# facebookresearch/KeypointNeRF

Measured on AMD Instinct MI355X. Metric: rendered rays/sec (64 coarse + 64 fine samples/ray), higher is better.
Workload: dtype f32 (dominant kernel: every fp32 operand as two fp16 pieces (22 bits, the residual formed exactly), three fp16-MFMA products per term set (hh hl lh: all terms above 2^-24 relative), fp32 accumulation; everything else fp32)

## Files before the change

### include/kpnerf.h

```cpp
#ifndef KPNERF_H
#define KPNERF_H

#include <stddef.h>
#include <stdint.h>

#ifdef __cplusplus
extern "C" {
#endif

#define KPN_ABI_VERSION 10
#define KPN_N_KPT 24
#define KPN_MAX_VIEWS 16

enum { KPN_OK = 0, KPN_EINVAL = -1, KPN_ELAUNCH = -2, KPN_EWORKSPACE = -3 };

int kpn_abi_version(void);
const char* kpn_last_error(void);
int kpn_is_device_build(void);

size_t kpn_plain_weight_floats(void);
size_t kpn_packed_weight_floats(void);
int kpn_pack_weights(const float* plain_host, float* packed_host);
int kpn_pack_weights_device(const float* plain_dev, float* packed_dev, void* stream);

// ... 31 lines not shown

int kpn_importance_sample(const float* contrib, const float* z, const float* u, int64_t n_rays, int32_t d_minus_2,
                          int32_t n_samples, float* samples_out, void* stream);

int kpn_rgba2out(const float* rgba, const float* z, int64_t n_rays, int32_t n_samples, float* color, float* depth,
                 float* alpha, float* contrib, float* sdf, void* stream);

int kpn_rgba2out_backward(const float* rgba, const float* z, int64_t n_rays, int32_t n_samples, const float* d_color,
                          const float* d_depth, const float* d_alpha, const float* d_sdf, float* d_rgba, void* stream);

size_t kpn_geo_rows_backward_workspace_bytes(int64_t n_points, int32_t n_views);
int kpn_geo_rows_backward(const kpn_scene_desc* desc, const void* scene_ws, const float* packed_weights, int64_t n_points,
                          const float* pts, uint32_t keep_mask, const float* d_x, float* d_plain, float* d_geo0,
                          float* d_geo1, void* workspace, size_t workspace_bytes, void* stream);

size_t kpn_query_backward_geometry_workspace_bytes(int64_t n_points, int32_t n_views);
int kpn_query_backward_geometry(const kpn_scene_desc* desc, const void* scene_ws, const float* packed_weights,
                                int64_t n_points, const float* pts, int32_t mode, uint32_t keep_mask, const float* noise,
                                float noise_std, const float* d_out, float* d_plain, float* d_geo0, float* d_geo1,
                                void* workspace, size_t workspace_bytes, void* stream);

size_t kpn_query_backward_workspace_bytes(int64_t n_points, int32_t n_views);
int kpn_query_backward(const kpn_scene_desc* desc, const void* scene_ws, const float* packed_weights, int64_t n_points,
                       const float* pts, const float* view, int32_t mode, uint32_t keep_mask, const float* noise,
                       float noise_std, const float* d_out, float* d_plain, float* d_geo0, float* d_geo1, float* d_tex,
                       void* workspace, size_t workspace_bytes, void* stream);

size_t kpn_geo_rows_backward_workspace_bytes_kpt(int64_t n_points, int32_t n_views);
int kpn_geo_rows_backward_kpt(const kpn_scene_desc* desc, const void* scene_ws, const float* packed_weights, int64_t n_points,
                              const float* pts, uint32_t keep_mask, const float* d_x, float* d_plain, float* d_geo0,
                              float* d_geo1, float* d_kpt3d, int32_t n_kpt, void* workspace, size_t workspace_bytes, void* stream);
size_t kpn_query_backward_workspace_bytes_kpt(int64_t n_points, int32_t n_views);
int kpn_query_backward_kpt(const kpn_scene_desc* desc, const void* scene_ws, const float* packed_weights, int64_t n_points,
                           const float* pts, const float* view, int32_t mode, uint32_t keep_mask, const float* noise,
                           float noise_std, const float* d_out, float* d_plain, float* d_geo0, float* d_geo1, float* d_tex,
                           float* d_kpt3d, int32_t n_kpt, void* workspace, size_t workspace_bytes, void* stream);

int kpn_set_geo_rows_mode(int32_t mode);
int kpn_get_geo_rows_mode(void);
int kpn_set_fuse_mode(int32_t mode);
int kpn_get_fuse_mode(void);
int kpn_set_density_first(int32_t mode);
int kpn_get_density_first(void);
int kpn_density_first_passes(int64_t* density_first, int64_t* fused, int32_t reset);
int kpn_density_stats(void* stream, int64_t* listed, int64_t* live, int32_t reset);
int kpn_packed_f16_range_check(const float* packed_weights_dev, void* stream, int32_t* beyond);
int kpn_set_range_guard(int32_t on);
int kpn_get_range_guard(void);
int kpn_range_guard_count(void* stream, int64_t* batches_host);

size_t kpn_query_workspace_bytes(int64_t n_points, int32_t n_views);
int kpn_query(const kpn_scene_desc* desc, const void* scene_ws, const float* packed_weights, int64_t n_points,
              const float* pts, const float* view, int32_t mode, float* out, uint8_t* valid, void* workspace,
              size_t workspace_bytes, void* stream);

typedef struct kpn_render_stages {
    float* z_coarse;
    float* rgba_coarse;
    float* z_fine;
    float* rgba_fine;
    float* dirs;
    float* cam_pos;
} kpn_render_stages;
typedef struct kpn_render_args {
    const float* K;
    const float* RT;
    const float* bounds;
    float znear, zfar;
    int32_t x0, y0, step, nx, ny;
    int32_t n_coarse, n_fine;
    int32_t fine;
    int32_t chunk_rays;
    float* tex_fg; float* depth; float* alpha;
    float* tex_fg_fine; float* depth_fine; float* alpha_fine; float* sdf;
    int32_t step_y;
    int32_t rows_kernel;
    int32_t fuse_kernel;
    const kpn_render_stages* stages;
} kpn_render_args;
enum { KPN_ROWS_DEFAULT = 0, KPN_ROWS_F32 = 1, KPN_ROWS_BF16X3 = 2, KPN_ROWS_F16X2 = 3 };
enum { KPN_FUSE_DEFAULT = 0, KPN_FUSE_F32 = 1, KPN_FUSE_F16X2 = 2 };

size_t kpn_render_workspace_bytes(const kpn_scene_desc* desc, const kpn_render_args* args);
int kpn_render_rays(const kpn_scene_desc* desc, const void* scene_ws, const float* packed_weights,
                    const kpn_render_args* args, void* workspace, size_t workspace_bytes, void* stream);

int kpn_pix_l1_loss(const float* src, const float* tar, int64_t n, float lambda, float* loss, float* d_src, void* scratch,
                    void* stream);
typedef struct kpn_train_loss_args {
    const float* tex;
    const float* tex_fine;
    const float* tar;
    const float* alpha;
    const float* alpha_fine;
    const float* tar_alpha;
    int64_t n;
    float l1_c, l1, l2, lp, mloss;
    int32_t reset_ticket;
    float* terms;
    float* d_tex;
    float* d_tex_fine;
    float* d_alpha;
    float* d_alpha_fine;
} kpn_train_loss_args;
size_t kpn_train_loss_workspace_bytes(int64_t n);
int kpn_train_loss(const kpn_train_loss_args* args, void* workspace, void* stream);
int kpn_frame_to_rgb8(const float* chw, int32_t height, int32_t width, int32_t bgr, uint8_t* hwc_out, void* stream);
int kpn_mse_psnr(const float* pred, const float* gt, int64_t n, double* out2, void* scratch, void* stream);
size_t kpn_ssim_scratch_bytes(int32_t crop_w, int32_t crop_h);
int kpn_ssim(const float* pred_chw, const float* gt_chw, int32_t height, int32_t width, int32_t x0, int32_t y0, int32_t crop_w,
             int32_t crop_h, double* out, void* scratch, void* stream);

int kpn_profile_enable(int32_t on);
int kpn_profile_collect(double* geo_rows_ms_host, int64_t* launches_host, int64_t* rows_host);
int kpn_profile_collect2(double* geo_rows_ms_host, int64_t* launches_host, int64_t* rows_host, int64_t* surplus_launches_host);
int kpn_profile_collect3(double* geo_rows_ms_host, int64_t* launches_host, int64_t* rows_host, int64_t* surplus_launches_host,
                         double* clock_ghz_host);
int kpn_bwd_profile_enable(int32_t on);
int kpn_bwd_profile_collect(double* ms5, int64_t* launches5, int64_t* rows, int64_t* kept_rows, int64_t* points);
size_t kpn_row_scratch_cap_bytes(void);
int kpn_set_row_scratch_cap_bytes(size_t bytes);

typedef struct kpn_train_args {
    const int32_t* pix;
    const float* u_coarse;
    const float* noise_coarse;
    const float* noise_fine;
    const float* u_fine;
    uint32_t keep_coarse;
    uint32_t keep_fine;
    float rand_noise_std;
} kpn_train_args;
int kpn_render_rays_train(const kpn_scene_desc* desc, const void* scene_ws, const float* packed_weights,
                          const kpn_render_args* args, const kpn_train_args* train, void* workspace,
                          size_t workspace_bytes, void* stream);

typedef struct kpn_render_grads {
    const float* d_tex_fg; const float* d_depth; const float* d_alpha;
    const float* d_tex_fg_fine; const float* d_depth_fine; const float* d_alpha_fine; const float* d_sdf;
} kpn_render_grads;
size_t kpn_render_rays_train_backward_workspace_bytes(const kpn_scene_desc* desc, const kpn_render_args* args);
int kpn_render_rays_train_backward(const kpn_scene_desc* desc, const void* scene_ws, const float* packed_weights,
                                   const kpn_render_args* args, const kpn_train_args* train, const kpn_render_grads* grads,
                                   float* d_plain, float* d_geo0, float* d_geo1, float* d_tex, void* workspace,
                                   size_t workspace_bytes, void* stream);

size_t kpn_render_rays_train_state_bytes(const kpn_scene_desc* desc, const kpn_render_args* args);
int kpn_render_rays_train_keep(const kpn_scene_desc* desc, const void* scene_ws, const float* packed_weights,
                               const kpn_render_args* args, const kpn_train_args* train, void* state, size_t state_bytes,
                               void* stream);
int kpn_render_rays_train_backward_kept(const kpn_scene_desc* desc, const void* scene_ws, const float* packed_weights,
                                        const kpn_render_args* args, const kpn_train_args* train, const kpn_render_grads* grads,
                                        float* d_plain, float* d_geo0, float* d_geo1, float* d_tex, void* state,
                                        size_t state_bytes, void* workspace, size_t workspace_bytes, void* stream);

size_t kpn_render_rays_train_backward_workspace_bytes_kpt(const kpn_scene_desc* desc, const kpn_render_args* args);
int kpn_render_rays_train_backward_kpt(const kpn_scene_desc* desc, const void* scene_ws, const float* packed_weights,
                                       const kpn_render_args* args, const kpn_train_args* train, const kpn_render_grads* grads,
                                       float* d_plain, float* d_geo0, float* d_geo1, float* d_tex, float* d_kpt3d, int32_t n_kpt,
                                       void* workspace, size_t workspace_bytes, void* stream);
int kpn_render_rays_train_backward_kept_kpt(const kpn_scene_desc* desc, const void* scene_ws, const float* packed_weights,
                                            const kpn_render_args* args, const kpn_train_args* train, const kpn_render_grads* grads,
                                            float* d_plain, float* d_geo0, float* d_geo1, float* d_tex, float* d_kpt3d,
                                            int32_t n_kpt, void* state, size_t state_bytes, void* workspace,
                                            size_t workspace_bytes, void* stream);

// ... 216 lines not shown
```

### keypointnerf_amd/csrc/api_backward.hip

```cpp
namespace {
const int64_t kBwdChunk = 262144;
static_assert(kBwdChunk <= 262144, "kUncappedPoints (query_layout) must cover a backward pass");
#ifndef KPN_GRAD_WORKERS
#define KPN_GRAD_WORKERS 512
#endif
const int kGradWorkers = kEmu ? 3 : KPN_GRAD_WORKERS;
const int kPartialUnits = 72;
struct BwdBufs { kpn_bwd_bufs B; kpn_fuse_bwd_bufs F; kpn_color_bufs C; };
enum { PART_GEO = 0, PART_FUSE, PART_DXROWS, PART_COLOR, PART_CMP };
const int kPartFull[5] = {0, 1, 1, 2, 2};
enum { U_X0 = 0, U_X1, U_X2, U_X3, U_D0, U_D1, U_D2, U_D3, U_XP, U_XH0, U_XH1, U_D20, U_D21, U_D22, U_DXROWS,
       U_XRD, U_XE1, U_XDIR, U_XBL, U_XB1, U_XA, U_XV10, U_XV11, U_XT33, U_XV20, U_XV21, U_XO0, U_XO1, U_XO2,
       U_DO2, U_DO1, U_DO0, U_DV21, U_DV20, U_DV11, U_DV10, U_DBL1, U_DBL0, U_DRE1, U_DRE0, U_DCMP, U_COUNT };
struct Dump { int id; size_t member; int ld; int part; };
#define D(id, member, ld, part) {U_##id, offsetof(BwdBufs, member), ld, PART_##part}
constexpr Dump kDumps[U_COUNT] = {
    D(X0, B.X0, KPN_LDX0, GEO), D(X1, B.X1, 128, GEO), D(X2, B.X2, KPN_LDX2, GEO), D(X3, B.X3, 128, GEO),
    D(D0, B.D0, 128, GEO), D(D1, B.D1, 128, GEO), D(D2, B.D2, 128, GEO), D(D3, B.D3, 64, GEO),
    D(XP, F.Xp, 128, FUSE), D(XH0, F.Xh0, 64, FUSE), D(XH1, F.Xh1, 64, FUSE), D(D20, F.D20, 64, FUSE), D(D21, F.D21, 64, FUSE), D(D22, F.D22, 2, FUSE),
    D(DXROWS, F.dxrows, 64, DXROWS),
    D(XRD, C.Xrd, 4, COLOR), D(XE1, C.Xe1, 16, COLOR), D(XDIR, C.Xdir, KPN_LD_XDIR, COLOR), D(XBL, C.Xbl, KPN_LD_XBL, COLOR), D(XB1, C.Xb1, 64, COLOR),
    D(XA, C.Xa, 32, COLOR), D(XV10, C.Xv10, 32, COLOR), D(XV11, C.Xv11, 32, COLOR), D(XT33, C.Xt33, 2, COLOR), D(XV20, C.Xv20, 32, COLOR),
    D(XV21, C.Xv21, 32, COLOR), D(XO0, C.Xo0, KPN_LD_XO0, COLOR), D(XO1, C.Xo1, 16, COLOR), D(XO2, C.Xo2, 8, COLOR),
    D(DO2, C.Do2, 2, COLOR), D(DO1, C.Do1, 8, COLOR), D(DO0, C.Do0, 16, COLOR), D(DV21, C.Dv21, 2, COLOR), D(DV20, C.Dv20, 32, COLOR),
// ... 97 lines not shown
    if (p.ws_bytes < L.total) return fail(KPN_EWORKSPACE, "backward workspace too small");
    const KptLayout K = kpt_layout(L.total, V);
    if (p.d_kpt) {
        KPN_REQUIRE(p.n_kpt >= 1 && p.n_kpt <= KPN_NKPT, "n_kpt in 1..24");
        if (p.ws_bytes < K.total) return fail(KPN_EWORKSPACE, "backward workspace too small for the keypoint gradient");
    }
    if (p.marched && p.N > L.chunk) return fail(KPN_EINVAL, "ray-marched backward pass too large");
    kpn_scene_dev sc = scene_dev(d, scene_ws);
    sc.keep = p.keep_mask;
    char* base = static_cast<char*>(p.ws);
    auto fp = [&](size_t off) { return reinterpret_cast<float*>(base + off); };
    int* count = reinterpret_cast<int*>(base + L.count);
    int64_t* rows_dev = reinterpret_cast<int64_t*>(base + L.count + 64);
    int* list = reinterpret_cast<int*>(base + L.list);
    BwdBufs u{};
    for (const Dump& m : kDumps) if (full >= kPartFull[m.part]) dump_slot(u, m) = fp(L.dump[m.id]);
    u.B.dgeo0 = p.d_geo0; u.B.dgeo1 = p.d_geo1;
    if (full == 2) {
        u.C.dtex = p.d_tex;
        u.C.dani = p.d_plain + kpn_plain_weight_floats() - 1;
        u.F.Dcmp = u.C.Dcmp;
    }
    const int blocks = field_grid_blocks();
    const uint32_t wgrad_keep = p.keep_mask | ~((V >= 32) ? 0xFFFFFFFFu : ((1u << V) - 1u));
    kpn_wgrad_jobs jobs[3], all;
    int gzmax[3];
    size_t partial_used = 0;
    bool overflow = false;
    auto queue_jobs = [&](int stage) {
        for (const WgradRow& r : kWgrad) {
            if (r.stage != stage) continue;
            const Dump &dy = kDumps[r.dY], &x = kDumps[r.X];
            const int cls = r.mv == 1 ? 0 : (r.mv == 2 ? 1 : 2);
            const int gz = (r.Kc + 63) / 64;
            kpn_wgrad_job j;
            j.dY = dump_slot(u, dy); j.X = dump_slot(u, x); j.ldy = dy.ld; j.M = r.M; j.ldx = x.ld; j.Kc = r.Kc; j.Kt = r.Kt;
            j.cmap = r.cmap; j.omap = r.omap; j.mv = r.mv;
            j.which = per_point(x) ? 1 : 0;
            j.V = per_point(x) ? 1 : V; j.keep = per_point(x) ? 0xFFFFFFFFu : wgrad_keep;
            j.partial = fp(L.partial) + partial_used;
            partial_used += (size_t)gz * kGradWorkers * r.mv * 2048;
            if (partial_used > (size_t)kPartialUnits * kGradWorkers * 2048 || all.n >= KPN_WGRAD_MAX_JOBS) { overflow = true; continue; }
            j.dbp = fp(L.dbp) + (size_t)all.n * kGradWorkers * 4 * 64;
            j.dW = p.d_plain + plain_w_off(r.layer);
            j.dB = p.d_plain + plain_b_off(r.layer);
            j.in_dim = plain_dims[r.layer][1];
            jobs[cls].j[jobs[cls].n++] = j;
            all.j[all.n++] = j;
            if (gz > gzmax[cls]) gzmax[cls] = gz;
        }
    };
    auto run_jobs = [&]() {
        if (jobs[0].n) KPN_LAUNCH(k_weight_grad<1>, dim3(kGradWorkers, jobs[0].n), dim3(64 * gzmax[0]), stream, jobs[0], (const int64_t*)rows_dev);
        if (jobs[1].n) KPN_LAUNCH(k_weight_grad<2>, dim3(kGradWorkers, jobs[1].n), dim3(64 * gzmax[1]), stream, jobs[1], (const int64_t*)rows_dev);
        if (jobs[2].n) KPN_LAUNCH(k_weight_grad<4>, dim3(kGradWorkers, jobs[2].n), dim3(64 * gzmax[2]), stream, jobs[2], (const int64_t*)rows_dev);
        int gz_all = gzmax[0] > gzmax[1] ? gzmax[0] : gzmax[1];
        if (gzmax[2] > gz_all) gz_all = gzmax[2];
        const int mv_all = jobs[2].n ? 4 : (jobs[1].n ? 2 : 1);
        if (all.n) KPN_LAUNCH(k_weight_grad_reduce, dim3((mv_all * 2048 + mv_all * 32 + 31) / 32, gz_all, all.n), dim3(256), stream, all,
                              (int)kGradWorkers);
    };
    if (p.d_kpt) {
        hipMemsetAsync(base + K.partial, 0, K.partial_bytes, (hipStream_t)stream);
        KPN_LAUNCH(k_kpt_grad_pack, grid1d(KPN_KG_WT_FLOATS, 256), dim3(256), stream, wp, fp(K.wt));
    }
    for (int64_t c0 = 0; c0 < p.N; c0 += L.chunk) {
        const int64_t n = (p.N - c0 < L.chunk) ? (p.N - c0) : L.chunk;
        const kpn_points ps = p.marched ? *p.marched
                                        : kpn_points{p.pts + c0 * 3, (p.view ? p.view : p.pts) + c0 * 3, nullptr, nullptr, nullptr, 1,
                                                     p.noise ? p.noise + c0 : nullptr, p.noise_std};
        jobs[0].n = jobs[1].n = jobs[2].n = all.n = 0; gzmax[0] = gzmax[1] = gzmax[2] = 0; partial_used = 0;
        hipMemsetAsync(count, 0, 8 * sizeof(int), (hipStream_t)stream);
        const int* vcount = count;
        float* xscr = full ? fp(L.xscr) : nullptr;
        if (p.fwd_query_ws && full) {
            const QueryLayout Q = query_layout(n, V);
            char* qb = static_cast<char*>(p.fwd_query_ws);
            vcount = reinterpret_cast<const int*>(qb + Q.count);
            list = reinterpret_cast<int*>(qb + Q.list);
            xscr = reinterpret_cast<float*>(qb + Q.xscr);
        } else {
            const int ppt = mask_points_per_thread(n);
            KPN_LAUNCH(k_mask_compact, grid1d(n, 256 * ppt), dim3(256), stream, sc, ps, n, 0, 1, ppt, wp + kpn_scalar_off(), (float*)nullptr,
                       (uint8_t*)nullptr, list, count);
        }
        KPN_LAUNCH(k_bwd_rows, dim3(1), dim3(1), stream, vcount, V, rows_dev);
        bwd_prof_pass(vcount, V, p.keep_mask, stream);
        if (full) {
            if (!p.fwd_query_ws) {
                KPN_BPROF(BP_ROWS_FWD);
                KPN_LAUNCH(k_geo_rows, dim3(blocks), dim3(256), stream, sc, ps, wp, (const int*)list, vcount, count + 1, xscr,
                           kpn_batch{0, 1 << 30});
            }
            if (full == 2) {
                KPN_BPROF(BP_COLOR_BWD);
                if (V <= 3)
                    KPN_LAUNCH(k_color_bwd<3>, dim3(blocks), dim3(256), stream, sc, ps, wp, (const int*)list, vcount, count + 4,
                               (const float*)xscr, p.d_out + c0 * 5, u.C);
                else
                    KPN_LAUNCH(k_color_bwd<KPN_MAXV>, dim3(blocks), dim3(256), stream, sc, ps, wp, (const int*)list, vcount, count + 4,
                               (const float*)xscr, p.d_out + c0 * 5, u.C);
            }
            if (full == 2) queue_jobs(ST_COLOR);
            {
                KPN_BPROF(BP_FUSE_BWD);
                KPN_LAUNCH(k_fuse_bwd, dim3(blocks), dim3(256), stream, sc, ps, wp, (const int*)list, vcount, count + 2,
                           (const float*)xscr, p.mode, p.d_out + c0 * 5, u.F);
            }
            queue_jobs(ST_LAYERS2);
            if (full == 2) queue_jobs(ST_COMPRESS);
        }
        {
            KPN_BPROF(BP_ROWS_BWD);
            KPN_LAUNCH(k_geo_rows_bwd, dim3(blocks), dim3(256), stream, sc, ps, wp, (const int*)list, vcount, count + 3,
                       full ? (const float*)u.F.dxrows : p.d_x + c0 * V * 64, full ? 1 : 0, u.B);
        }
        if (p.d_kpt) {
            const kpn_kpt_grad_args ka{u.B.D0, u.B.X0, fp(K.wt), reinterpret_cast<double*>(base + K.partial), p.n_kpt, wgrad_keep};
            KPN_LAUNCH(k_kpt_grad, dim3(kKptWorkers, V), dim3(256), stream, sc, ps, (const int*)list, vcount, ka);
        }
        queue_jobs(ST_LAYERS1);
        if (overflow) return fail(KPN_EWORKSPACE, "weight-gradient scratch too small (internal)");
        {
            KPN_BPROF(BP_WGRAD);
            run_jobs();
        }
    }
    if (p.d_kpt)
        KPN_LAUNCH(k_kpt_grad_finish, dim3(p.n_kpt), dim3(256), stream, sc, (const double*)reinterpret_cast<double*>(base + K.partial),
                   (int)kKptWorkers, p.d_kpt);
    return check_launch("field backward");
}
}

extern "C" size_t kpn_geo_rows_backward_workspace_bytes(int64_t N, int32_t V) { return bwd_workspace_bytes(N, V, 0); }

extern "C" int kpn_geo_rows_backward(const kpn_scene_desc* d, const void* scene_ws, const float* wp, int64_t N,
                                     const float* pts, uint32_t keep_mask, const float* d_x, float* d_plain, float* d_geo0,
                                     float* d_geo1, void* ws, size_t ws_bytes, void* stream) {
    if (int e = check_desc(d)) return e;
    KPN_REQUIRE(N >= 0 && N < (1ll << 31), "point count out of range");
    if (N == 0) return KPN_OK;
    KPN_REQUIRE(scene_ws && wp && pts && d_x && d_plain && d_geo0 && d_geo1 && ws, "null pointer");
    BackwardPass p;
    p.N = N; p.pts = pts; p.keep_mask = keep_mask; p.d_x = d_x;
    p.d_plain = d_plain; p.d_geo0 = d_geo0; p.d_geo1 = d_geo1; p.ws = ws; p.ws_bytes = ws_bytes;
    return run_backward(d, scene_ws, wp, p, stream);
}

extern "C" size_t kpn_geo_rows_backward_workspace_bytes_kpt(int64_t N, int32_t V) { return bwd_workspace_bytes_kpt(N, V, 0); }

extern "C" int kpn_geo_rows_backward_kpt(const kpn_scene_desc* d, const void* scene_ws, const float* wp, int64_t N,
                                         const float* pts, uint32_t keep_mask, const float* d_x, float* d_plain, float* d_geo0,
                                         float* d_geo1, float* d_kpt3d, int32_t n_kpt, void* ws, size_t ws_bytes, void* stream) {
    if (int e = check_desc(d)) return e;
    KPN_REQUIRE(N >= 0 && N < (1ll << 31), "point count out of range");
    KPN_REQUIRE(n_kpt >= 1 && n_kpt <= KPN_NKPT, "n_kpt in 1..24");
    if (N == 0) return KPN_OK;
    KPN_REQUIRE(scene_ws && wp && pts && d_x && d_plain && d_geo0 && d_geo1 && d_kpt3d && ws, "null pointer");
    BackwardPass p;
    p.N = N; p.pts = pts; p.keep_mask = keep_mask; p.d_x = d_x;
    p.d_plain = d_plain; p.d_geo0 = d_geo0; p.d_geo1 = d_geo1; p.ws = ws; p.ws_bytes = ws_bytes;
    p.d_kpt = d_kpt3d; p.n_kpt = n_kpt;
    return run_backward(d, scene_ws, wp, p, stream);
}

extern "C" size_t kpn_query_backward_geometry_workspace_bytes(int64_t N, int32_t V) { return bwd_workspace_bytes(N, V, 1); }
// ... 52 lines not shown
```

### keypointnerf_amd/csrc/api_field.hip

```cpp
namespace {
struct Setting { long long value = -1; template <class Init> long long get(Init init) { if (value < 0) value = init(); return value; } };
bool env_flag(const char* name) { const char* e = getenv(name); return e && atoi(e) != 0; }
#ifdef KPN_SIMT_EMU
const bool kEmu = true;
#else
const bool kEmu = false;
#endif
Setting g_row_scratch_cap, g_geo_rows_mode, g_fuse_mode, g_density_first, g_range_guard, g_no_pool;

size_t row_scratch_cap_bytes() {
    return (size_t)g_row_scratch_cap.get([] {
        const char* e = getenv("KPN_ROW_SCRATCH_MIB");
        return (long long)((e ? (size_t)atoll(e) : (size_t)(kEmu ? 1 : 3072)) << 20);
    });
}
const int kMaxBatches = 60;
const size_t kCounterBytes = 2048;
static_assert((8 + 8 * kMaxBatches) * sizeof(int) <= kCounterBytes && kCounterBytes % 256 == 0, "counter block");
const int64_t kUncappedPoints = kEmu ? 2048 : 262144;
struct QueryLayout { size_t count, list, live, xscr, total; int tiles_cap, nbatch; };
#ifndef KPN_DEFAULT_GEO_ROWS_MODE
#define KPN_DEFAULT_GEO_ROWS_MODE 3
#endif
int geo_rows_mode() { return (int)g_geo_rows_mode.get([] { return (long long)KPN_DEFAULT_GEO_ROWS_MODE; }); }
// ... 43 lines not shown
    return &g_density_hint[0];
#endif
}
long long g_density_first_passes[2] = {0, 0};
bool density_first_now() {
    const int m = density_first();
    if (m != 2) return m == 1;
    DensityHint* hnt = density_hint();
    if (!hnt) return false;
#ifndef KPN_SIMT_EMU
    if (!hnt->pinned) return hnt->split;
    const unsigned long long now[2] = {hnt->pinned[0], hnt->pinned[1]};
#else
    const unsigned long long now[2] = {kpn_density_counts[0], kpn_density_counts[1]};
#endif
    const bool was_reset = now[0] < hnt->seen[0];
    const unsigned long long d0 = was_reset ? now[0] : now[0] - hnt->seen[0], d1 = was_reset ? now[1] : now[1] - hnt->seen[1];
    if (d0 > 0 && d1 <= d0) {
        hnt->avg[0] = 0.5 * hnt->avg[0] + (double)d0;
        hnt->avg[1] = 0.5 * hnt->avg[1] + (double)d1;
        hnt->split = (hnt->avg[0] - hnt->avg[1]) >= (double)kDensityFirstDeadFraction * hnt->avg[0];
        hnt->seen[0] = now[0]; hnt->seen[1] = now[1];
    }
    return hnt->split;
}
void density_hint_refresh(void* stream) {
#ifndef KPN_SIMT_EMU
    if (density_first() != 2 || stream_is_capturing(stream)) return;
    DensityHint* hnt = density_hint();
    if (!hnt) return;
    if (!hnt->pinned) {
        void* hp = nullptr;
        if (hipHostMalloc(&hp, 2 * sizeof(unsigned long long), hipHostMallocDefault) != hipSuccess) { (void)hipGetLastError(); return; }
        hnt->pinned = static_cast<unsigned long long*>(hp);
        hnt->pinned[0] = hnt->pinned[1] = 0;
    }
    void* dp = nullptr;
    if (hipGetSymbolAddress(&dp, HIP_SYMBOL(kpn_density_counts)) != hipSuccess) { (void)hipGetLastError(); return; }
    (void)hipMemcpyAsync(hnt->pinned, dp, 2 * sizeof(unsigned long long), hipMemcpyDeviceToHost, (hipStream_t)stream);
#else
    (void)stream;
#endif
}
int pair_grid_blocks() {
#ifdef KPN_SIMT_EMU
    return 8;
#else
    static int blocks = [] {
        int dev = 0, cus = 0;
        if (hipGetDevice(&dev) != hipSuccess || hipDeviceGetAttribute(&cus, hipDeviceAttributeMultiprocessorCount, dev) != hipSuccess || cus <= 0) cus = 256;
        return cus;
    }();
    return blocks;
#endif
}
int fuse_grid_blocks() { return kEmu ? 4 : 256; }
int records_grid_blocks() { return kEmu ? 8 : 2048; }
static inline int mask_points_per_thread(int64_t N) {
    const int64_t min_groups = kEmu ? 2 : 2048;
    int ppt = KPN_MASK_PPT;
    while (ppt > 1 && N / (256 * (int64_t)ppt) < min_groups) ppt >>= 1;
    return ppt;
}
int range_guard() { return (int)g_range_guard.get([] { return (long long)!env_flag("KPN_NO_RANGE_GUARD"); }); }
#ifndef KPN_SIMT_EMU
__device__ int kpn_redone_batches;
#else
static int kpn_redone_batches;
#endif
int* redone_counter() {
#ifndef KPN_SIMT_EMU
    void* p = nullptr;
    if (hipGetSymbolAddress(&p, HIP_SYMBOL(kpn_redone_batches)) != hipSuccess) return nullptr;
    return static_cast<int*>(p);
#else
    return &kpn_redone_batches;
#endif
}

struct FieldPass {
    kpn_points points; int64_t N = 0; int mode = 0;
    float* out = nullptr; uint8_t* valid = nullptr; void* ws = nullptr;
    bool lean = false, keep_rows = false, allow_pool = false; int rows_sel = 0, fuse_sel = 0;
};
struct FieldLaunch { const kpn_scene_dev& sc; const kpn_points& ps; const float* wp; int *list, *count, *live; float* xscr; void* stream; };
kpn_batch make_batch(int index, int tiles_cap, bool pool, int cond = KPN_RUN_ALWAYS, int* bad = nullptr, int* redone = nullptr) {
    return kpn_batch{index, tiles_cap, cond, bad, redone, pool ? 1 : 0, nullptr};
}

void launch_rows(const FieldLaunch& f, int rows_mode, int* tickets, const kpn_batch& batch) {
    if (rows_mode >= 2)
        kpn_internal_launch_geo_rows_pair(rows_mode, pair_grid_blocks(), f.stream, &f.sc, &f.ps, f.wp, f.list, f.count, tickets, f.xscr, &batch);
    else
        KPN_LAUNCH(k_geo_rows, dim3(field_grid_blocks()), dim3(256), f.stream, f.sc, f.ps, f.wp, (const int*)f.list, (const int*)f.count, tickets, f.xscr, batch);
}
void launch_records(const FieldLaunch& f, const kpn_batch& batch) {
    kpn_internal_launch_row_records(records_grid_blocks(), f.stream, &f.sc, &f.ps, f.wp, f.list, f.count, f.xscr, &batch);
}
bool use_h3(const kpn_scene_dev& sc) { return sc.V == 3 && (sc.keep & 7u) == 7u && !env_flag("KPN_NO_FUSE_H3"); }
void launch_fuse(const FieldLaunch& f, int fmode, int* tickets, int mode, float* out, const kpn_batch& batch, int zero_skip) {
    auto* kernel = fmode != 1 ? k_fuse_color : (use_h3(f.sc) ? k_fuse_color_h3 : k_fuse_color_h);
    KPN_LAUNCH(kernel, dim3(fuse_grid_blocks()), dim3(512), f.stream, f.sc, f.ps, f.wp, (const int*)f.list, (const int*)f.count, tickets, (const float*)f.xscr, mode, 0, out, batch, zero_skip);
}
void launch_density_first(const FieldLaunch& f, int* tickets, float* out, const kpn_batch& batch) {
    const int fblocks = fuse_grid_blocks();
    KPN_LAUNCH(k_density_h, dim3(fblocks), dim3(512), f.stream, f.sc, f.ps, f.wp, (const int*)f.list, (const int*)f.count, tickets, f.xscr, f.live, out, batch);
    kpn_internal_launch_row_records_live(records_grid_blocks(), f.stream, &f.sc, &f.ps, f.wp, f.list, f.count, tickets, f.live, f.xscr, &batch);
    auto* colour = use_h3(f.sc) ? k_colour_h3 : k_colour_h;
    KPN_LAUNCH(colour, dim3(fblocks), dim3(512), f.stream, f.sc, f.ps, f.wp, (const int*)f.list, (const int*)f.count, tickets, (const float*)f.xscr, f.live, out, batch);
}

int selected_rows_mode(int sel) { return sel == KPN_ROWS_F32 ? 0 : (sel == KPN_ROWS_BF16X3 ? 2 : (sel == KPN_ROWS_F16X2 ? 3 : geo_rows_mode())); }
int selected_fuse_mode(int sel) { return sel == KPN_FUSE_F32 ? 0 : (sel == KPN_FUSE_F16X2 ? 1 : fuse_mode()); }

int run_field(const kpn_scene_dev& sc, const float* wp, const FieldPass& p, void* stream) {
    const kpn_points& ps = p.points;
    const int rmode = selected_rows_mode(p.rows_sel);
    const int fmode = !p.out ? 0 : selected_fuse_mode(p.fuse_sel);
    const bool pool = p.allow_pool && !p.keep_rows && p.out && pool_layout_selected() && rmode >= 2;
    const QueryLayout L = query_layout(p.N, sc.V, pool);
    char* base = static_cast<char*>(p.ws);
    int* count = reinterpret_cast<int*>(base + L.count);
    const FieldLaunch f{sc, ps, wp, reinterpret_cast<int*>(base + L.list), count, reinterpret_cast<int*>(base + L.live),
                        reinterpret_cast<float*>(base + L.xscr), stream};
    hipMemsetAsync(count, 0, kCounterBytes, (hipStream_t)stream);
    const int ppt = mask_points_per_thread(p.N);
    KPN_LAUNCH(k_mask_compact, grid1d(p.N, 256 * ppt), dim3(256), stream, sc, ps, p.N, p.mode, (int)p.lean, ppt, wp + kpn_scalar_off(), p.out, p.valid, f.list, count);
    if (p.keep_rows && L.nbatch > 1) return fail(KPN_EWORKSPACE, "a pass whose rows a backward call reads again must fit the row scratch");
    const bool guard = range_guard() && p.out && (rmode == 3 || fmode == 1);
    int* redone = guard ? redone_counter() : nullptr;
    const int safe_rmode = rmode == 3 ? 2 : rmode;
    auto guarded = [&](bool f16) { return guard && f16 ? KPN_RUN_IF_SAFE : KPN_RUN_ALWAYS; };
    const int zero_skip = (p.lean && !p.keep_rows && !env_flag("KPN_NO_ZERO_SKIP")) ? 1 : 0;
    const bool eligible = zero_skip && p.mode == 1 && ps.noise == nullptr && pool && fmode == 1;
    const bool split = eligible && density_first_now();
    if (eligible) ++g_density_first_passes[split ? 0 : 1];
    for (int b = 0; b < L.nbatch; ++b) {
        int* slots = count + 8 + 8 * b;
        int* bad = guard ? slots + 6 : nullptr;
        kpn_batch b_rows = make_batch(b, L.tiles_cap, pool, guarded(rmode == 3), bad);
        {
            KPN_FPROF(b_rows, rmode >= 2, count, sc.V);
            launch_rows(f, rmode, slots + 0, b_rows);
        }
        if (rmode >= 2 && !split) launch_records(f, make_batch(b, L.tiles_cap, pool));
        if (!p.out) continue;
        const kpn_batch b_fuse = make_batch(b, L.tiles_cap, pool, guarded(fmode == 1), bad);
        if (split) launch_density_first(f, slots, p.out, b_fuse);
        else launch_fuse(f, fmode, slots, p.mode, p.out, b_fuse, zero_skip);
        if (guard) {
            const kpn_batch r_rows = make_batch(b, L.tiles_cap, pool, KPN_RUN_IF_UNSAFE, bad);
            launch_rows(f, safe_rmode, slots + 4, r_rows);
            if (split) launch_records(f, r_rows);
            launch_fuse(f, 0, slots + 4, p.mode, p.out, make_batch(b, L.tiles_cap, pool, KPN_RUN_IF_UNSAFE, bad, redone), zero_skip);
        }
    }
    if (eligible) density_hint_refresh(stream);
    return check_launch("field query");
}
}

extern "C" int kpn_set_geo_rows_mode(int32_t mode) {
    KPN_REQUIRE(mode == 0 || mode == 2 || mode == 3, "mode must be 0 (fp32 MFMA), 2 (three bf16 pieces) or 3 (two fp16 pieces); mode 1 is not part of the library");
    g_geo_rows_mode.value = mode;
    return KPN_OK;
}
extern "C" int kpn_get_geo_rows_mode(void) { return geo_rows_mode(); }
extern "C" int kpn_set_fuse_mode(int32_t mode) {
    KPN_REQUIRE(mode == 0 || mode == 1, "mode must be 0 (fp32 MFMA) or 1 (two fp16 pieces per operand)");
    g_fuse_mode.value = mode;
    return KPN_OK;
}
extern "C" int kpn_get_fuse_mode(void) { return fuse_mode(); }
extern "C" int kpn_density_stats(void* stream, int64_t* listed_host, int64_t* live_host, int32_t reset) {
    KPN_REQUIRE(listed_host && live_host, "null pointer");
    unsigned long long v[2] = {0, 0};
#ifndef KPN_SIMT_EMU
    void* p = nullptr;
    if (hipGetSymbolAddress(&p, HIP_SYMBOL(kpn_density_counts)) != hipSuccess) return fail(KPN_ELAUNCH, "no density counters in this module");
    if (hipMemcpyAsync(v, p, sizeof(v), hipMemcpyDeviceToHost, (hipStream_t)stream) != hipSuccess ||
        (reset && hipMemsetAsync(p, 0, sizeof(v), (hipStream_t)stream) != hipSuccess) ||
        hipStreamSynchronize((hipStream_t)stream) != hipSuccess) return fail(KPN_ELAUNCH, "could not read the density counters");
#else
    (void)stream;
    v[0] = kpn_density_counts[0]; v[1] = kpn_density_counts[1];
    if (reset) kpn_density_counts[0] = kpn_density_counts[1] = 0;
#endif
    *listed_host = (int64_t)v[0];
    *live_host = (int64_t)v[1];
    return KPN_OK;
}
#if defined(KPN_PRECISION_PROBE) && !defined(KPN_SIMT_EMU)
extern "C" int kpn_internal_probe_set_mask_pair(unsigned long long m);
extern "C" int kpn_probe_set_mask(unsigned long long m) {
    if (hipMemcpyToSymbol(HIP_SYMBOL(kpn_probe_mask_dev), &m, sizeof(m)) != hipSuccess) return fail(KPN_ELAUNCH, "probe mask");
    if (kpn_internal_probe_set_mask_pair(m)) return fail(KPN_ELAUNCH, "probe mask (pair unit)");
    return hipDeviceSynchronize() == hipSuccess ? KPN_OK : KPN_ELAUNCH;
}
#endif
extern "C" int kpn_density_first_passes(int64_t* density_first_host, int64_t* fused_host, int32_t reset) {
    KPN_REQUIRE(density_first_host && fused_host, "null pointer");
    *density_first_host = g_density_first_passes[0];
    *fused_host = g_density_first_passes[1];
    if (reset) g_density_first_passes[0] = g_density_first_passes[1] = 0;
    return KPN_OK;
}
extern "C" int kpn_set_density_first(int32_t mode) {
    KPN_REQUIRE(mode >= 0 && mode <= 2, "mode must be 0 (fused per-point kernel), 1 (density first) or 2 (auto)");
    g_density_first.value = mode;
    return KPN_OK;
// ... 47 lines not shown
```

### keypointnerf_amd/csrc/api_render.hip

```cpp
namespace {
struct RayBlock { size_t cam_pos, dirs, nearv, farv; };
struct RayView { float *cam_pos, *dirs, *nearv, *farv; };
RayBlock carve_rays(Carver& c, int64_t R) { return {c.take(64), c.take((size_t)R * 3 * 4), c.take((size_t)R * 4), c.take((size_t)R * 4)}; }
struct ChunkBlock { size_t zc, zf, rgba_c, rgba_f, contrib, query_c, query_f; };
struct ChunkView { float *zc, *zf, *rgba_c, *rgba_f, *contrib; char *query_c, *query_f; };
ChunkBlock carve_chunk(Carver& c, int64_t C, int64_t Sc, int64_t Sfull, bool train) {
    ChunkBlock k{};
    k.zc = c.take((size_t)C * Sc * 4); k.zf = c.take((size_t)C * Sfull * 4);
    if (train) {
        k.rgba_c = c.take((size_t)C * Sc * 5 * 4); k.rgba_f = c.take((size_t)C * Sfull * 5 * 4);
        k.contrib = c.take((size_t)C * (Sfull > 8 ? Sfull : 8) * 4);
    } else {
        k.rgba_c = k.rgba_f = c.take((size_t)C * Sfull * 5 * 4);
        c.o += 256;
    }
    return k;
}
template <class T = float> T* at(void* base, size_t off) { return reinterpret_cast<T*>(static_cast<char*>(base) + off); }
RayView ray_view(void* base, const RayBlock& r) { return {at(base, r.cam_pos), at(base, r.dirs), at(base, r.nearv), at(base, r.farv)}; }
ChunkView chunk_view(void* base, const ChunkBlock& k) {
    return {at(base, k.zc), at(base, k.zf), at(base, k.rgba_c), at(base, k.rgba_f), at(base, k.contrib), at<char>(base, k.query_c), at<char>(base, k.query_f)};
}

struct RenderLayout { RayBlock rays; ChunkBlock k; size_t rgba_n, zn, src, color, depth, alpha, sdf, total; int64_t chunk; };
int64_t pick_chunk(const kpn_scene_desc* d, const kpn_render_args* a) {
    const int64_t R = (int64_t)a->nx * a->ny;
    int64_t c = a->chunk_rays;
    if (c <= 0) {
        const int64_t cmax = 262144;
        const int64_t npass = (R + cmax - 1) / cmax;
        c = ((R + npass - 1) / npass + 63) / 64 * 64;
    }
    return c < R ? c : R;
}
RenderLayout render_layout(const kpn_scene_desc* d, const kpn_render_args* a) {
    RenderLayout L;
    const int64_t C = pick_chunk(d, a);
    const int64_t Sfull = a->n_coarse + (a->fine ? a->n_fine : 0);
    Carver c;
    L.chunk = C;
    L.rays = carve_rays(c, (int64_t)a->nx * a->ny);
    L.k = carve_chunk(c, C, a->n_coarse, Sfull, false);
    L.rgba_n = L.k.rgba_c + align_up((size_t)C * a->n_coarse * 5 * 4, 256);
    L.zn = c.take((size_t)C * (a->fine ? a->n_fine : 0) * 4);
    L.src = c.take((size_t)C * Sfull * sizeof(int16_t));
    L.k.contrib = c.take((size_t)C * a->n_coarse * 4);
    L.color = c.take((size_t)C * 3 * 4);
    L.depth = c.take((size_t)C * 4);
    L.alpha = c.take((size_t)C * 4);
    L.sdf = c.take((size_t)C * 4);
    {
        const size_t qa = query_layout(C * Sfull, d->n_views, false).total, qb = query_layout(C * Sfull, d->n_views, pool_layout_selected()).total;
        L.k.query_c = L.k.query_f = c.take(qa > qb ? qa : qb);
    }
    L.total = c.o;
    return L;
}
int check_render(const kpn_render_args* a) {
    KPN_REQUIRE(a != nullptr, "render args null");
    KPN_REQUIRE(a->K && a->RT && a->bounds, "null camera/bounds");
    KPN_REQUIRE(a->nx > 0 && a->ny > 0 && a->step > 0 && a->step_y >= 0, "bad pixel grid");
    KPN_REQUIRE(a->rows_kernel >= 0 && a->rows_kernel <= KPN_ROWS_F16X2 && a->fuse_kernel >= 0 && a->fuse_kernel <= KPN_FUSE_F16X2, "bad kernel selection");
    KPN_REQUIRE(a->n_coarse >= 3 && a->n_coarse <= 128, "sample_per_ray_c must be in [3,128]");
    KPN_REQUIRE(!a->fine || (a->n_fine >= 1 && a->n_fine <= 128), "sample_per_ray_f must be in [1,128]");
    KPN_REQUIRE((int64_t)a->nx * a->ny < (1ll << 31), "too many rays");
    return KPN_OK;
}
int check_train(const kpn_scene_desc* d, const kpn_render_args* a, const kpn_train_args* t, bool need_fine) {
    KPN_REQUIRE(t != nullptr, "train args null");
    KPN_REQUIRE(a->fine || !need_fine, "the train branch renders coarse + fine (dr_kwargs.fine)");
    KPN_REQUIRE(t->pix && t->u_coarse, "train args: pix and u_coarse are required");
    KPN_REQUIRE(!a->fine || t->u_fine, "train args: u_fine is required when fine");
    KPN_REQUIRE(t->rand_noise_std == 0.0f || (t->noise_coarse && (!a->fine || t->noise_fine)), "train args: noise tensors missing");
    KPN_REQUIRE((t->keep_coarse & ((1u << d->n_views) - 1u)) && (t->keep_fine & ((1u << d->n_views) - 1u)),
                "train args: view dropout must keep at least one view (reference src/model.py:744)");
    return KPN_OK;
}
}

__global__ void k_store_planar(int64_t r0, int64_t n, int64_t R, int C, const float* __restrict__ src, float* __restrict__ dst) {
    const int64_t i = (int64_t)blockIdx.x * blockDim.x + threadIdx.x;
    if (i >= n * C) return;
    const int64_t r = i / C;
    const int c = (int)(i - r * C);
    dst[(int64_t)c * R + r0 + r] = src[i];
}
__global__ void k_load_planar(int64_t r0, int64_t n, int64_t R, int C, const float* __restrict__ src, float* __restrict__ dst) {
    const int64_t i = (int64_t)blockIdx.x * blockDim.x + threadIdx.x;
    if (i >= n * C) return;
    const int64_t r = i / C;
    const int c = (int)(i - r * C);
    dst[i] = src ? src[(int64_t)c * R + r0 + r] : 0.0f;
}
struct PlanarChunk {
    void* stream; int64_t r0, n, R;
    void store(float* dst, const float* src, int C) const {
        if (dst) KPN_LAUNCH(k_store_planar, grid1d(n * C, 256), dim3(256), stream, r0, n, R, C, src, dst);
    }
    void load(float* dst, const float* src, int C) const {
        KPN_LAUNCH(k_load_planar, grid1d(n * C, 256), dim3(256), stream, r0, n, R, C, src, dst);
    }
};

extern "C" size_t kpn_render_workspace_bytes(const kpn_scene_desc* d, const kpn_render_args* a) {
    if (check_desc(d) != KPN_OK || check_render(a) != KPN_OK) return 0;
    return render_layout(d, a).total;
}

static void launch_fine_samples(void* stream, int64_t n, int Sc, int Sf, const float* zc, const float* contrib,
                                const float* u, float* zf, float* znew, int16_t* src) {
    const bool small = Sc <= 64 && Sf <= 64;
    const int64_t per = 4 * KPN_FINE_GROUP(small);
    const dim3 grid((unsigned)((n + per - 1) / per < 8192 ? (n + per - 1) / per : 8192));
    if (small)
        KPN_LAUNCH(k_fine_samples_w<true>, grid, dim3(256), stream, n, Sc, Sf, zc, contrib, u, zf, znew, src);
    else
        KPN_LAUNCH(k_fine_samples_w<false>, grid, dim3(256), stream, n, Sc, Sf, zc, contrib, u, zf, znew, src);
}

static void launch_make_rays(void* stream, const kpn_render_args* a, const int* pix, int step_y, const RayView& rays) {
    KPN_LAUNCH(k_make_rays, grid1d((int64_t)a->nx * a->ny, 256), dim3(256), stream, a->K, a->RT, a->znear, a->zfar, a->bounds, (int)a->x0, (int)a->y0,
               (int)a->step, step_y, (int)a->nx, (int)a->ny, pix, rays.dirs, rays.cam_pos, rays.nearv, rays.farv);
}

static int render_impl(const kpn_scene_desc* d, const void* scene_ws, const float* wp, const kpn_render_args* a,
                       const kpn_train_args* t, void* ws, size_t ws_bytes, void* stream) {
    if (int e = check_desc(d)) return e;
    if (int e = check_render(a)) return e;
    KPN_REQUIRE(scene_ws && wp && ws, "null pointer");
    if (t) if (int e = check_train(d, a, t, false)) return e;
    const RenderLayout L = render_layout(d, a);
    if (ws_bytes < L.total) return fail(KPN_EWORKSPACE, "render workspace too small");
    const RayView rays = ray_view(ws, L.rays);
    const ChunkView k = chunk_view(ws, L.k);
    float *rgba_n = at(ws, L.rgba_n), *zn = at(ws, L.zn), *color = at(ws, L.color), *depth = at(ws, L.depth), *alpha = at(ws, L.alpha), *sdf = at(ws, L.sdf);
    int16_t* src = at<int16_t>(ws, L.src);
    kpn_scene_dev sc = scene_dev(d, scene_ws);
    const int64_t R = (int64_t)a->nx * a->ny;
    const int Sc = a->n_coarse, Sf = a->fine ? a->n_fine : 0, Sfull = Sc + Sf;
    const float std_ = t ? t->rand_noise_std : 0.0f;
    launch_make_rays(stream, a, t ? (const int*)t->pix : (const int*)nullptr, (int)(a->step_y > 0 ? a->step_y : a->step), rays);
    for (int64_t r0 = 0; r0 < R; r0 += L.chunk) {
        const int64_t n = (R - r0) < L.chunk ? (R - r0) : L.chunk;
        const float* dirs = rays.dirs + r0 * 3;
        const PlanarChunk pl{stream, r0, n, R};
        KPN_LAUNCH(k_coarse_z, grid1d(n * Sc, 256), dim3(256), stream, n, Sc, (const float*)(rays.nearv + r0),
                   (const float*)(rays.farv + r0), t ? t->u_coarse + r0 * Sc : (const float*)nullptr, k.zc);
        const bool reuse = (t == nullptr) && a->fine && !env_flag("KPN_NO_COARSE_REUSE");
        auto field = [&](const float* z, int S, const float* noise, float* out) {
            FieldPass p;
            p.points = kpn_points{nullptr, nullptr, rays.cam_pos, dirs, z, S, noise, std_};
            p.N = n * S; p.mode = 1; p.out = out; p.ws = k.query_c; p.lean = true; p.allow_pool = t == nullptr;
            p.rows_sel = a->rows_kernel; p.fuse_sel = a->fuse_kernel;
            return run_field(sc, wp, p, stream);
        };
        sc.keep = t ? t->keep_coarse : 0xFFFFFFFFu;
        if (int e = field(k.zc, Sc, std_ != 0.0f ? t->noise_coarse + r0 * Sc : nullptr, k.rgba_c)) return e;
        if (int e = kpn_rgba2out(k.rgba_c, k.zc, n, Sc, color, depth, alpha, k.contrib, sdf, stream)) return e;
        const kpn_render_stages* st = a->stages;
        auto copy_out = [&](float* dst, const float* src_, size_t floats) {
            (void)hipMemcpyAsync(dst, src_, floats * sizeof(float), hipMemcpyDeviceToDevice, (hipStream_t)stream);
        };
        if (st && st->dirs) copy_out(st->dirs + r0 * 3, dirs, (size_t)n * 3);
        if (st && st->cam_pos && r0 == 0) copy_out(st->cam_pos, rays.cam_pos, 3);
        if (st && st->z_coarse) copy_out(st->z_coarse + r0 * Sc, k.zc, (size_t)n * Sc);
        if (st && st->rgba_coarse) copy_out(st->rgba_coarse + r0 * Sc * 5, k.rgba_c, (size_t)n * Sc * 5);
        pl.store(a->tex_fg, color, 3);
        pl.store(a->depth, depth, 1);
        pl.store(a->alpha, alpha, 1);
        if (!a->fine) continue;
        launch_fine_samples(stream, n, Sc, Sf, k.zc, k.contrib, t ? t->u_fine + r0 * Sf : (const float*)nullptr, k.zf, reuse ? zn : nullptr,
                            reuse ? src : nullptr);
        sc.keep = t ? t->keep_fine : 0xFFFFFFFFu;
        if (reuse) {
            if (int e = field(zn, Sf, nullptr, rgba_n)) return e;
            if (int e = rgba2out_merged(k.rgba_c, rgba_n, src, k.zf, n, Sc, Sf, color, depth, alpha, sdf, stream)) return e;
        } else {
            if (int e = field(k.zf, Sfull, std_ != 0.0f ? t->noise_fine + r0 * Sfull : nullptr, k.rgba_f)) return e;
            if (int e = kpn_rgba2out(k.rgba_f, k.zf, n, Sfull, color, depth, alpha, nullptr, sdf, stream)) return e;
        }
        if (st && st->z_fine) copy_out(st->z_fine + r0 * Sfull, k.zf, (size_t)n * Sfull);
        if (st && st->rgba_fine) {
            if (reuse) KPN_LAUNCH(k_merge_rgba, grid1d(n * Sfull, 256), dim3(256), stream, n, Sfull, Sc, (const float*)k.rgba_c, (const float*)rgba_n,
                                  (const int16_t*)src, st->rgba_fine + r0 * Sfull * 5);
            else copy_out(st->rgba_fine + r0 * Sfull * 5, k.rgba_f, (size_t)n * Sfull * 5);
        }
        pl.store(a->tex_fg_fine, color, 3);
        pl.store(a->depth_fine, depth, 1);
        pl.store(a->alpha_fine, alpha, 1);
        pl.store(a->sdf, sdf, 1);
    }
    return check_launch("kpn_render_rays");
}

extern "C" int kpn_render_rays(const kpn_scene_desc* d, const void* scene_ws, const float* wp, const kpn_render_args* a,
                               void* ws, size_t ws_bytes, void* stream) {
    return render_impl(d, scene_ws, wp, a, nullptr, ws, ws_bytes, stream);
}
extern "C" int kpn_render_rays_train(const kpn_scene_desc* d, const void* scene_ws, const float* wp, const kpn_render_args* a,
                                     const kpn_train_args* t, void* ws, size_t ws_bytes, void* stream) {
    KPN_REQUIRE(t != nullptr, "train args null");
    return render_impl(d, scene_ws, wp, a, t, ws, ws_bytes, stream);
}

namespace {
struct TrainBwdLayout { RayBlock rays; ChunkBlock k; size_t scratch, g3, g1a, g1b, g1c, drgba_c, drgba_f, bwd, total; int64_t chunk; };
TrainBwdLayout train_bwd_layout(const kpn_scene_desc* d, const kpn_render_args* a) {
    TrainBwdLayout L;
    const int64_t R = (int64_t)a->nx * a->ny;
    const int64_t Sfull = a->n_coarse + a->n_fine;
    int64_t C = a->chunk_rays > 0 ? a->chunk_rays : kBwdChunk / Sfull;
    if (C * Sfull > kBwdChunk) C = kBwdChunk / Sfull;
    if (C > R) C = R;
    L.chunk = C;
    Carver c;
    L.rays = carve_rays(c, R);
    L.k = carve_chunk(c, C, a->n_coarse, Sfull, true);
    L.scratch = c.take((size_t)C * 8 * 4);
    L.g3 = c.take((size_t)C * 3 * 4); L.g1a = c.take((size_t)C * 4); L.g1b = c.take((size_t)C * 4); L.g1c = c.take((size_t)C * 4);
    L.drgba_c = c.take((size_t)C * a->n_coarse * 5 * 4); L.drgba_f = c.take((size_t)C * Sfull * 5 * 4);
    L.k.query_c = L.k.query_f = c.take(query_layout(C * Sfull, d->n_views).total);
    L.bwd = c.take(bwd_layout(C * Sfull, d->n_views, 2).total);
    L.total = c.o;
    return L;
}

struct TrainStateLayout { RayBlock rays; size_t chunk0; ChunkBlock k; size_t chunk_bytes, total; int64_t chunk, nchunks; };
TrainStateLayout train_state_layout(const kpn_scene_desc* d, const kpn_render_args* a) {
    TrainStateLayout S;
    const int64_t R = (int64_t)a->nx * a->ny, C = train_bwd_layout(d, a).chunk;
    const int64_t Sfull = a->n_coarse + a->n_fine;
    S.chunk = C; S.nchunks = (R + C - 1) / C;
    Carver c;
    S.rays = carve_rays(c, R);
    S.chunk0 = c.o;
    c = Carver();
    S.k = carve_chunk(c, C, a->n_coarse, Sfull, true);
    S.k.query_c = c.take(query_layout(C * a->n_coarse, d->n_views).total);
    S.k.query_f = c.take(query_layout(C * Sfull, d->n_views).total);
    S.chunk_bytes = c.o;
    S.total = S.chunk0 + S.chunk_bytes * (size_t)S.nchunks;
    return S;
}

struct TrainPass { bool fine; kpn_points ps; uint32_t keep; float *z, *rgba; char* query; };
struct TrainChunk { int64_t r0, n; ChunkView v; PlanarChunk pl; TrainPass coarse, fine; };
struct TrainCall {
    const kpn_scene_desc* d; const void* scene_ws; const float* wp; const kpn_render_args* a; const kpn_train_args* t;
    const kpn_render_grads* g; float *d_plain, *d_geo0, *d_geo1, *d_tex;
    void *state, *ws, *stream;
    TrainBwdLayout L; TrainStateLayout S;
    kpn_scene_dev sc; int64_t R; int Sc, Sf, Sfull; RayView rays;
    float* d_kpt = nullptr; int n_kpt = 0;
    size_t bwd_bytes() const { return d_kpt ? kpt_layout(L.total - L.bwd, d->n_views).total : L.total - L.bwd; }
    int begin(size_t state_bytes, size_t ws_bytes, bool forward_only) {
        if (int e = check_desc(d)) return e;
        if (int e = check_render(a)) return e;
        KPN_REQUIRE(a->rows_kernel == KPN_ROWS_DEFAULT && a->fuse_kernel == KPN_FUSE_DEFAULT,
                    "the train branch takes the process-wide kernel selection: rows_kernel / fuse_kernel must be 0");
        KPN_REQUIRE(scene_ws && wp, "null pointer");
        if (int e = check_train(d, a, t, true)) return e;
        if (!forward_only) KPN_REQUIRE(g && d_plain && d_geo0 && d_geo1 && d_tex && ws, "gradient pointers / workspace null");
        if (forward_only) KPN_REQUIRE(state != nullptr, "state null");
        L = train_bwd_layout(d, a);
        S = train_state_layout(d, a);
        if (d_kpt) KPN_REQUIRE(n_kpt >= 1 && n_kpt <= KPN_NKPT, "n_kpt in 1..24");
        if (!forward_only && ws_bytes < L.bwd + bwd_bytes()) return fail(KPN_EWORKSPACE, "train backward workspace too small");
        if (state && state_bytes < S.total) return fail(KPN_EWORKSPACE, "train state too small");
        sc = scene_dev(d, scene_ws);
// ... 138 lines not shown
```

### keypointnerf_amd/csrc/api_scene.hip

```cpp
namespace {
struct SceneLayout { size_t table, rgbm, geo0, geo1, tex, flags, total; };
SceneLayout scene_layout(const kpn_scene_desc* d) {
    SceneLayout L;
    Carver c;
    L.table = c.take((size_t)d->n_views * KPN_TBL_STRIDE, 64);
    L.rgbm = c.take((size_t)d->n_views * d->src_h * d->src_w * 4, 64);
    L.geo0 = c.take((size_t)d->n_views * d->geo0_h * d->geo0_w * 64, 64);
    L.geo1 = c.take((size_t)d->n_views * d->geo1_h * d->geo1_w * 8, 64);
    L.tex = c.take((size_t)d->n_views * d->tex_h * d->tex_w * 8, 64);
    L.flags = c.take((size_t)KPN_SCENE_FLAG_FLOATS, 64);
    L.total = c.o;
    return L;
}
int check_desc(const kpn_scene_desc* d) {
    KPN_REQUIRE(d != nullptr, "scene desc is null");
    KPN_REQUIRE(d->n_views >= 1 && d->n_views <= KPN_MAX_VIEWS, "n_views out of range");
    KPN_REQUIRE(d->src_h > 1 && d->src_w > 1 && d->geo0_h > 1 && d->geo0_w > 1 && d->geo1_h > 1 && d->geo1_w > 1 &&
                d->tex_h > 1 && d->tex_w > 1, "map sizes must be > 1");
    KPN_REQUIRE((int64_t)d->src_h * d->src_w <= INT32_MAX && (int64_t)d->geo0_h * d->geo0_w <= INT32_MAX &&
                (int64_t)d->geo1_h * d->geo1_w <= INT32_MAX && (int64_t)d->tex_h * d->tex_w <= INT32_MAX, "map too large");
    KPN_REQUIRE(d->zfar > d->znear && d->nml_scale > 0.0f && d->sigma > 0.0f, "bad scalar parameters");
    KPN_REQUIRE(d->KRT && d->extrin && d->kpt3d && d->img && d->geo0 && d->geo1 && d->tex, "null scene tensor");
    KPN_REQUIRE(d->disable_fg_mask || d->fg_mask, "fg_mask is null");
    return KPN_OK;
}
kpn_scene_dev scene_dev(const kpn_scene_desc* d, const void* ws) {
    const SceneLayout L = scene_layout(d);
    const float* base = static_cast<const float*>(ws);
    kpn_scene_dev s;
    s.V = d->n_views; s.H = d->src_h; s.W = d->src_w;
    s.g0h = d->geo0_h; s.g0w = d->geo0_w; s.g1h = d->geo1_h; s.g1w = d->geo1_w; s.th = d->tex_h; s.tw = d->tex_w;
    s.disable_fg_mask = d->disable_fg_mask;
    s.znear = d->znear; s.zfar = d->zfar; s.nml_scale = d->nml_scale;
    s.two_sigma2 = (float)(2.0 * ((double)d->sigma * (double)d->sigma));
    s.keep = 0xFFFFFFFFu;
    s.table = base + L.table; s.rgbm = base + L.rgbm; s.geo0 = base + L.geo0; s.geo1 = base + L.geo1; s.tex = base + L.tex;
    s.flags = base + L.flags;
    return s;
}
}

extern "C" size_t kpn_scene_workspace_bytes(const kpn_scene_desc* d) {
    if (check_desc(d) != KPN_OK) return 0;
    return scene_layout(d).total * sizeof(float);
}

extern "C" int kpn_scene_layout(const kpn_scene_desc* d, size_t offsets[6]) {
    if (int e = check_desc(d)) return e;
    KPN_REQUIRE(offsets != nullptr, "offsets is null");
    const SceneLayout L = scene_layout(d);
    offsets[0] = L.table; offsets[1] = L.rgbm; offsets[2] = L.geo0; offsets[3] = L.geo1; offsets[4] = L.tex; offsets[5] = L.flags;
    return KPN_OK;
}

extern "C" int kpn_scene_prepare(const kpn_scene_desc* d, void* scene_ws, void* stream) {
    return kpn_scene_prepare_kpt(d, KPN_NKPT, scene_ws, stream);
}

extern "C" int kpn_scene_prepare_kpt(const kpn_scene_desc* d, int32_t n_kpt, void* scene_ws, void* stream) {
    if (int e = check_desc(d)) return e;
    KPN_REQUIRE(n_kpt >= 1 && n_kpt <= KPN_NKPT, "n_kpt out of range: the field kernels hold 1..24 keypoints (KPN_N_KPT)");
    KPN_REQUIRE(scene_ws != nullptr, "scene workspace is null");
    const SceneLayout L = scene_layout(d);
    float* base = static_cast<float*>(scene_ws);
    const int V = d->n_views;
    float* flags = base + L.flags;
    KPN_LAUNCH(k_scene_table, dim3(V), dim3(128), stream, V, (int)n_kpt, d->KRT, d->extrin, d->kpt3d, base + L.table, flags);
    const int HW = d->src_h * d->src_w;
    const int ptiles = (HW + KPN_PACK_PIX - 1) / KPN_PACK_PIX;
    KPN_LAUNCH(k_pack_rgbm, dim3(V * ptiles), dim3(256), stream, HW, ptiles, d->img,
               d->disable_fg_mask ? (const uint8_t*)nullptr : d->fg_mask, base + L.rgbm, flags);
    auto vec = [](const float* p, int hw) { return (hw % 4 == 0 && reinterpret_cast<uintptr_t>(p) % 16 == 0) ? 1 : 0; };
    const int hw0 = d->geo0_h * d->geo0_w, hw1 = d->geo1_h * d->geo1_w, hwt = d->tex_h * d->tex_w;
    const int t0 = (hw0 + KPN_NHWC_TILE / 64 - 1) / (KPN_NHWC_TILE / 64), t1 = (hw1 + KPN_NHWC_TILE / 8 - 1) / (KPN_NHWC_TILE / 8),
              tt = (hwt + KPN_NHWC_TILE / 8 - 1) / (KPN_NHWC_TILE / 8);
    KPN_LAUNCH(k_nchw_to_nhwc<64>, dim3(V * t0), dim3(256), stream, hw0, t0, vec(d->geo0, hw0), d->geo0, base + L.geo0, flags);
    KPN_LAUNCH(k_nchw_to_nhwc<8>, dim3(V * t1), dim3(256), stream, hw1, t1, vec(d->geo1, hw1), d->geo1, base + L.geo1, flags);
    KPN_LAUNCH(k_nchw_to_nhwc<8>, dim3(V * tt), dim3(256), stream, hwt, tt, vec(d->tex, hwt), d->tex, base + L.tex, flags);
    return check_launch("kpn_scene_prepare");
}

extern "C" int kpn_ray_bbox_intersection(const float* bounds, const float* orig, const float* direct, int64_t R,
                                         float* near_o, float* far_o, uint8_t* hit_o, void* stream) {
    KPN_REQUIRE(bounds && orig && direct && near_o && far_o && hit_o, "null pointer");
    KPN_REQUIRE(R >= 0, "negative ray count");
    if (R == 0) return KPN_OK;
    KPN_LAUNCH(k_ray_bbox, grid1d(R, 256), dim3(256), stream, R, bounds, orig, direct, near_o, far_o, hit_o);
    return check_launch("kpn_ray_bbox_intersection");
}

extern "C" int kpn_make_rays(const float* K, const float* RT, float znear, float zfar, const float* bounds, int32_t x0,
                             int32_t y0, int32_t step, int32_t nx, int32_t ny, float* dirs, float* cam_pos,
                             float* near_o, float* far_o, void* stream) {
    KPN_REQUIRE(K && RT && bounds && dirs && cam_pos && near_o && far_o, "null pointer");
    KPN_REQUIRE(nx > 0 && ny > 0 && step > 0, "bad pixel grid");
    KPN_LAUNCH(k_make_rays, grid1d((int64_t)nx * ny, 256), dim3(256), stream, K, RT, znear, zfar, bounds, (int)x0, (int)y0,
               (int)step, (int)step, (int)nx, (int)ny, (const int*)nullptr, dirs, cam_pos, near_o, far_o);
    return check_launch("kpn_make_rays");
}

extern "C" int kpn_importance_sample(const float* contrib, const float* z, const float* u, int64_t R, int32_t Dm2,
                                     int32_t n, float* out, void* stream) {
    KPN_REQUIRE(contrib && z && out, "null pointer");
    KPN_REQUIRE(Dm2 >= 1 && Dm2 + 1 <= KPN_IS_MAXD, "bin count out of range (<= 128)");
    KPN_REQUIRE(n >= 1 && R >= 0, "bad sizes");
    if (R == 0) return KPN_OK;
    KPN_LAUNCH(k_importance, grid1d(R, 64), dim3(64), stream, R, (int)Dm2, (int)n, contrib, z, u, out);
    return check_launch("kpn_importance_sample");
}

static void launch_rgba2out(void* stream, int64_t R, int S, const float* rgba, const float* z, float* color, float* depth,
                            float* alpha, float* contrib, float* sdf, const int16_t* src, const float* rgba_new, int Sc) {
    const int64_t blocks = (R + 3) / 4;
    const dim3 grid((unsigned)(blocks < 8192 ? blocks : 8192));
    const int per = (S + 63) / 64;
    if (per <= 1) KPN_LAUNCH(k_rgba2out<1>, grid, dim3(256), stream, R, S, rgba, z, color, depth, alpha, contrib, sdf, src, rgba_new, Sc);
    else if (per <= 2) KPN_LAUNCH(k_rgba2out<2>, grid, dim3(256), stream, R, S, rgba, z, color, depth, alpha, contrib, sdf, src, rgba_new, Sc);
    else if (per <= 4) KPN_LAUNCH(k_rgba2out<4>, grid, dim3(256), stream, R, S, rgba, z, color, depth, alpha, contrib, sdf, src, rgba_new, Sc);
    else KPN_LAUNCH(k_rgba2out<KPN_MAX_PER_LANE>, grid, dim3(256), stream, R, S, rgba, z, color, depth, alpha, contrib, sdf, src, rgba_new, Sc);
}

extern "C" int kpn_rgba2out(const float* rgba, const float* z, int64_t R, int32_t S, float* color, float* depth,
                            float* alpha, float* contrib, float* sdf, void* stream) {
    KPN_REQUIRE(rgba && z && color && depth && alpha && sdf, "null pointer");
    KPN_REQUIRE(S >= 1 && S <= 64 * KPN_MAX_PER_LANE, "samples per ray out of range (<= 512)");
    if (R <= 0) return R == 0 ? KPN_OK : fail(KPN_EINVAL, "negative ray count");
    launch_rgba2out(stream, R, (int)S, rgba, z, color, depth, alpha, contrib, sdf, nullptr, nullptr, 0);
    return check_launch("kpn_rgba2out");
}
static int rgba2out_merged(const float* rgba_c, const float* rgba_n, const int16_t* src, const float* z, int64_t R, int Sc, int Sf,
                           float* color, float* depth, float* alpha, float* sdf, void* stream) {
    launch_rgba2out(stream, R, Sc + Sf, rgba_c, z, color, depth, alpha, nullptr, sdf, src, rgba_n, Sc);
    return check_launch("kpn_render_rays");
}

extern "C" int kpn_rgba2out_backward(const float* rgba, const float* z, int64_t R, int32_t S, const float* d_color,
                                     const float* d_depth, const float* d_alpha, const float* d_sdf, float* d_rgba, void* stream) {
    KPN_REQUIRE(rgba && z && d_rgba, "null pointer");
    KPN_REQUIRE(S >= 1, "bad sample count");
    if (R <= 0) return R == 0 ? KPN_OK : fail(KPN_EINVAL, "negative ray count");
    const int per = (int)((S + 63) / 64);
    const dim3 wgrid = grid1d(R * 64, 256);
    if (per <= 1) KPN_LAUNCH(k_rgba2out_bwd_w<1>, wgrid, dim3(256), stream, R, (int)S, rgba, z, d_color, d_depth, d_alpha, d_sdf, d_rgba);
    else if (per <= 2) KPN_LAUNCH(k_rgba2out_bwd_w<2>, wgrid, dim3(256), stream, R, (int)S, rgba, z, d_color, d_depth, d_alpha, d_sdf, d_rgba);
    else if (per <= 4) KPN_LAUNCH(k_rgba2out_bwd_w<4>, wgrid, dim3(256), stream, R, (int)S, rgba, z, d_color, d_depth, d_alpha, d_sdf, d_rgba);
    else if (per <= 8) KPN_LAUNCH(k_rgba2out_bwd_w<8>, wgrid, dim3(256), stream, R, (int)S, rgba, z, d_color, d_depth, d_alpha, d_sdf, d_rgba);
    else KPN_LAUNCH(k_rgba2out_bwd, grid1d(R, 64), dim3(64), stream, R, (int)S, rgba, z, d_color, d_depth, d_alpha, d_sdf, d_rgba);
    return check_launch("kpn_rgba2out_backward");
}
```

### keypointnerf_amd/csrc/field_kernels.hip

```cpp
#include "kpn_device.h"
#include "kpn_field_shared.h"

#define KPN_MASK_PPT 8
__global__ __launch_bounds__(256) void k_mask_compact(kpn_scene_dev sc, kpn_points ps, int64_t N, int mode, int lean, int ppt,
                                                      const float* __restrict__ wscalars, float* __restrict__ out,
                                                      uint8_t* __restrict__ valid, int* __restrict__ list,
                                                      int* __restrict__ count) {
    __shared__ unsigned long long mask_s[KPN_MASK_PPT][4];
    __shared__ int off_s[KPN_MASK_PPT][4];
    const int lane = threadIdx.x & 63, w = threadIdx.x >> 6;
    const int64_t n0 = (int64_t)blockIdx.x * 256 * ppt + threadIdx.x;
    for (int k = 0; k < ppt; ++k) {
        const int64_t n = n0 + (int64_t)k * 256;
        int is_valid = 0;
        if (n < N) {
            float P[3], D[3];
            kpn_get_point<true>(ps, n, P, D);
            int all_in = 1, all_fg = 1;
            float acc[3] = {0.f, 0.f, 0.f};
            const float pu = 1.0f / (float)sc.V;
            const size_t HW = (size_t)sc.H * sc.W;
            for (int v = 0; v < sc.V; ++v) {
                const float* tb = sc.table + (size_t)v * KPN_TBL_STRIDE;
                const kpn_proj q = kpn_project<true>(tb, P[0], P[1], P[2], sc);
                all_in &= q.in;
                if (lean && !all_in) break;
                const kpn_taps tp = kpn_make_taps<true>(q.xn, q.yn, sc.H, sc.W);
                const float4 s = kpn_tap4<true>(sc.rgbm + (size_t)v * HW * 4, 4, 0, tp);
                if (!sc.disable_fg_mask) all_fg &= (s.w > 0.1f);
                if (lean && !all_fg) break;
                acc[0] = KADD(acc[0], KMUL(s.x, pu)); acc[1] = KADD(acc[1], KMUL(s.y, pu)); acc[2] = KADD(acc[2], KMUL(s.z, pu));
            }
            is_valid = all_in && all_fg && ((sc.keep & ((1u << sc.V) - 1u)) != 0u);
            if (valid) valid[n] = (uint8_t)is_valid;
            if (!is_valid && out) {
                float* o = out + n * 5;
                if (mode == 1) { o[0] = 0.0f; o[1] = 0.1f / sc.nml_scale; }
                else { o[0] = wscalars[1]; o[1] = wscalars[2]; }
                o[2] = lean ? 0.0f : acc[0]; o[3] = lean ? 0.0f : acc[1]; o[4] = lean ? 0.0f : acc[2];
            }
        }
        const unsigned long long m = __ballot(is_valid);
        if (lane == 0) mask_s[k][w] = m;
    }
    __syncthreads();
    if (threadIdx.x == 0) {
        int total = 0;
        for (int k = 0; k < ppt; ++k)
            for (int j = 0; j < 4; ++j) { off_s[k][j] = total; total += __popcll(mask_s[k][j]); }
        const int base = total ? atomicAdd(count, total) : 0;
        for (int k = 0; k < ppt; ++k)
            for (int j = 0; j < 4; ++j) off_s[k][j] += base;
    }
    __syncthreads();
    for (int k = 0; k < ppt; ++k) {
        const unsigned long long m = mask_s[k][w];
        if ((m >> lane) & 1ull) list[off_s[k][w] + __popcll(m & ((1ull << lane) - 1ull))] = (int)(n0 + (int64_t)k * 256);
    }
}

__global__ __launch_bounds__(256, 2) void k_geo_rows(kpn_scene_dev sc, kpn_points ps, const float* __restrict__ wp,
                                                     const int* __restrict__ list, const int* __restrict__ count_ptr,
                                                     int* __restrict__ tickets, float* __restrict__ xscr, kpn_batch batch) {
    const int lane = threadIdx.x & 63;
    const int p = lane & 31, h = lane >> 5;
    const int wave = (blockIdx.x * blockDim.x + threadIdx.x) >> 6;
    const int nwaves = (gridDim.x * blockDim.x) >> 6;
    if (!kpn_batch_gate(batch, sc, wp)) return;
    const int count = *count_ptr;
    const int ntiles = (count + KPN_TILE - 1) / KPN_TILE;
    int t0, t1;
    if (!kpn_batch_range(batch, ntiles, t0, t1)) return;
    const int nwork = (t1 - t0) * sc.V;
    __shared__ __attribute__((aligned(16))) float bias_s[4][128];
    {
        const int segs[4] = {SEG_G1_0A, SEG_G1_1, SEG_G1_2, SEG_G1_3};
        for (int i = threadIdx.x; i < 4 * 128; i += blockDim.x) {
            const int sg = i >> 7, k = i & 127;
            bias_s[sg][k] = k < kpn_seg_bfloats(segs[sg]) ? wp[kpn_seg_boff(segs[sg]) + k] : 0.0f;
        }
    }
    __syncthreads();

    (void)wave; (void)nwaves;
    for (;;) {
        int wi = 0;
        if (lane == 0) wi = atomicAdd(tickets + 0, 1);
        wi = __shfl(wi, 0);
        if (wi >= nwork) break;
        const int tr = wi / sc.V, v = wi - tr * sc.V;
        int ci = (t0 + tr) * KPN_TILE + p;
        if (ci >= count) ci = count - 1;
        const int64_t n = list[ci];
        float P[3], D[3];
        kpn_get_point(ps, n, P, D);
        const float* tb = sc.table + (size_t)v * KPN_TBL_STRIDE;
        const kpn_proj q = kpn_project(tb, P[0], P[1], P[2], sc);
        if (!((sc.keep >> v) & 1u)) {
            float4 rec0, rec1;
            kpn_row_record(sc, ps, n, tb, v, h, rec0, rec1);
            float4* dst = reinterpret_cast<float4*>(xscr) + ((size_t)wi * KPN_ROW_SLABS) * 64 + lane;
#pragma unroll
            for (int k = 0; k < 8; ++k) dst[k * 64] = make_float4(0.f, 0.f, 0.f, 0.f);
            dst[8 * 64] = rec0;
            dst[9 * 64] = rec1;
            continue;
        }

        kpn_f32x16 a0[4];
        {
            const float* E = tb + KPN_TBL_EXT;
            const float cx = RADD(kpn_dot3(P[0], P[1], P[2], E[0], E[1], E[2]), E[3]);
            const float cy = RADD(kpn_dot3(P[0], P[1], P[2], E[4], E[5], E[6]), E[7]);
            const float cz = RADD(kpn_dot3(P[0], P[1], P[2], E[8], E[9], E[10]), E[11]);
            const float* kc = tb + KPN_TBL_KCAM + (12 * h) * 3;
            kpn_load_bias<4>(bias_s[0], h, a0);
            kpn_mfma_layer<84, 4, 7>(wp + kpn_seg_woff(SEG_G1_0A), lane, [&](auto gi, float (&x)[7]) {
                constexpr int j = decltype(gi)::value;
                const float dx = RSUB(cx, kc[j * 3 + 0]), dy = RSUB(cy, kc[j * 3 + 1]), dz = RSUB(cz, kc[j * 3 + 2]);
                const float d2 = RADD(RADD(RMUL(dx, dx), RMUL(dy, dy)), RMUL(dz, dz));
                const float w = kpn_fast_exp(-d2 / sc.two_sigma2);
                float s1, c1;
                kpn_sincos_pi(dz, s1, c1);
                const float s2 = 2.0f * s1 * c1, c2 = 1.0f - 2.0f * s1 * s1;
                const float s4 = 2.0f * s2 * c2, c4 = 1.0f - 2.0f * s2 * s2;
                x[0] = dz * w;
// ... 615 lines not shown
```

### keypointnerf_amd/csrc/geo_rows_pair_kernels.hip

```cpp

#ifndef KPN_H2_LOOKAHEAD
#define KPN_H2_LOOKAHEAD true
#endif
#ifdef KPN_SIMT_EMU
#define KPN_H2_PIN_ACC(v) ((void)0)
#else
#define KPN_H2_PIN_ACC(v) asm volatile("" : "+a"(v))
#endif
struct kpn_sc_bf16x3 {
    static constexpr int NP = 3, NPROD = 6, NSLICE = 6;
    static constexpr int pa(int pr) { return pr == 2 || pr == 3 ? 1 : (pr == 5 ? 2 : 0); }
    static constexpr int pb(int pr) { return pr == 1 || pr == 3 ? 1 : (pr == 4 ? 2 : 0); }
    static constexpr int hseg_base() { return kpn_hseg_off(0); }
    static constexpr float out_up = 1.0f, out_down = 1.0f;
    static constexpr bool PREFETCH = false;
    static constexpr int WBUF = 1;
    static __device__ __forceinline__ kpn_f32x16 mfma(kpn_f32x4 a, kpn_u32x4 b, kpn_f32x16 c);
};
struct kpn_sc_f16x2 {
    static constexpr int NP = 2, NPROD = KPN_F16_PRODUCTS, NSLICE = KPN_F16_PRODUCTS == 3 ? 3 : 4;
    static constexpr int pa(int pr) { return NPROD == 3 ? (pr == 2 ? 1 : 0) : pr >> 1; }
    static constexpr int pb(int pr) { return NPROD == 3 ? (pr == 1 ? 1 : 0) : pr & 1; }
    static constexpr int hseg_base() { return kpn_fseg_off(0); }
    static constexpr float out_up = KPN_F16_ROW_SCALE, out_down = 1.0f / KPN_F16_ROW_SCALE;
// ... 225 lines not shown
            acc[t][k] = SC::mfma(wa[wsel][SC::pa(prd)][k], x[t][SC::pb(prd)], acc[t][k]);
            KPN_H2_PIN_ACC(acc[t][k]);
        } else {
            constexpr int mm = m - 2 * NPROD * H0, prd = mm / (2 * H1), k = (mm / 2) % H1, t = mm % 2;
            acc[t][H0 + k] = SC::mfma(wb[wsel][SC::pa(prd)][k], x[t][SC::pb(prd)], acc[t][H0 + k]);
            KPN_H2_PIN_ACC(acc[t][H0 + k]);
        }
    };
    auto slice = [&](auto sn, int b, auto ti, auto ji, auto qi) {
        constexpr int t = decltype(ti)::value, j = decltype(ji)::value, q = decltype(qi)::value;
        constexpr bool act = decltype(sn)::value < ACT;
        if constexpr (!act && q < 3) stage_fn(sn, ti, ji, qi);
        kpn_h2_slice<SC, act, q, j>(pr, xp[b][t], [&]() { return val_fn(sn, ti, kpn_ic<2 * j>{}); }, [&]() { return val_fn(sn, ti, kpn_ic<2 * j + 1>{}); });
    };
    load_virtual(kpn_ic<0>{}, kpn_ic<0>{}); load_virtual(kpn_ic<0>{}, kpn_ic<1>{});
    if constexpr (WBUF == 2) { load_virtual(kpn_ic<1>{}, kpn_ic<0>{}); load_virtual(kpn_ic<1>{}, kpn_ic<1>{}); }
    if constexpr (HAVE0) {
#pragma unroll
        for (int t = 0; t < 2; ++t)
#pragma unroll
            for (int pc = 0; pc < NP; ++pc) xp[0][t][pc] = x0[t][pc];
    } else {
        kpn_static_for<0, 8>([&](auto pi) {
            constexpr int t = decltype(pi)::value % 2, j = decltype(pi)::value / 2;
            kpn_static_for<0, NSLICE>([&](auto qi) { slice(kpn_ic<0>{}, 0, kpn_ic<t>{}, kpn_ic<j>{}, qi); });
        });
    }
    KPN_SCHED_BARRIER();
    kpn_static_for<0, KS16>([&](auto si) {
        constexpr int s = decltype(si)::value;
        constexpr int cur = s & 1, nxt = cur ^ 1;
#ifdef KPN_PRECISION_PROBE
        if constexpr (NP == 2) {
            constexpr int lid = KS16 == 16 ? 0 : (KS16 == 9 ? 2 : (NOB == 2 ? 3 : 1));
            constexpr int grp = SMAP::at(s) < 12 ? 4 : 5;
            const bool drop_b = KPN_PROBE(lid, 0) || (lid == 0 && KPN_PROBE(grp, 0));
            const bool drop_a = KPN_PROBE(lid, 1) || (lid == 0 && KPN_PROBE(grp, 1));
            if (drop_b) { xp[cur][0][1] = kpn_u32x4{0u, 0u, 0u, 0u}; xp[cur][1][1] = kpn_u32x4{0u, 0u, 0u, 0u}; }
            if (drop_a) {
#pragma unroll
                for (int k = 0; k < H0; ++k) wa[wsel(s)][1][k] = kpn_f32x4{0.f, 0.f, 0.f, 0.f};
#pragma unroll
                for (int k = 0; k < H1; ++k) wb[wsel(s)][1][k] = kpn_f32x4{0.f, 0.f, 0.f, 0.f};
            }
        }
#endif
        kpn_static_for<0, MF>([&](auto mi) {
            constexpr int m = decltype(mi)::value;
            mfma(mi, kpn_ic<wsel(s)>{}, xp[cur]);
            if constexpr (s + 1 < KS16) {
                kpn_static_for<0, SPG>([&](auto ri) {
                    constexpr int k = m * SPG + decltype(ri)::value, pair = k / NSLICE;
                    slice(kpn_ic<s + 1>{}, nxt, kpn_ic<pair % 2>{}, kpn_ic<pair / 2>{}, kpn_ic<k % NSLICE>{});
                });
                if constexpr (m == 2 * NPROD * H0 - 1) load_virtual(kpn_ic<s + WBUF>{}, kpn_ic<0>{});
                if constexpr (m == MF - 1) load_virtual(kpn_ic<s + WBUF>{}, kpn_ic<1>{});
            } else {
                tail_fn(mi);
                if constexpr (NEXT && m >= MF / 2) {
                    kpn_static_for<0, 2 * SPG>([&](auto ri) {
                        constexpr int k = (m - MF / 2) * 2 * SPG + decltype(ri)::value, pair = k / NSLICE, t = pair % 2, j = pair / 2;
                        auto v0 = [&]() { return next_fn(kpn_ic<t>{}, kpn_ic<2 * j>{}); };
                        auto v1 = [&]() { return next_fn(kpn_ic<t>{}, kpn_ic<2 * j + 1>{}); };
                        kpn_h2_slice<SC, true, k % NSLICE, j>(pr, xn[t], v0, v1);
                    });
                }
            }
            KPN_SCHED_BARRIER();
        });
    });
}

#ifndef KPN_H2_L0_INTERLEAVE
#define KPN_H2_L0_INTERLEAVE 0
#endif
#ifndef KPN_H2_L0_AHEAD
#define KPN_H2_L0_AHEAD 2
#endif
struct kpn_h2_l0_order {
    static constexpr int at(int p) { return KPN_H2_L0_INTERLEAVE ? ((p % 4 == 3) ? 12 + p / 4 : p - p / 4) : p; }
};
#ifdef KPN_H2_TIMING
__device__ unsigned long long kpn_h2_cycles[8];
#define KPN_H2_STAMP(i) do { const unsigned long long now_ = clock64(); if (blockIdx.x == 3 && threadIdx.x == 64) atomicAdd(&kpn_h2_cycles[i], now_ - stamp_); stamp_ = now_; } while (0)
#else
#define KPN_H2_STAMP(i) ((void)0)
#endif
#ifndef KPN_SIMT_EMU
#ifdef KPN_H2_NUM_VGPR
#ifndef KPN_H2_WAVES_PER_SIMD
#define KPN_H2_WAVES_PER_SIMD 1
#endif
#define KPN_H2_BOUNDS __launch_bounds__(256, KPN_H2_WAVES_PER_SIMD) __attribute__((amdgpu_num_vgpr(KPN_H2_NUM_VGPR)))
#else
#define KPN_H2_BOUNDS __launch_bounds__(256, 1)
#endif
#else
#define KPN_H2_BOUNDS
#endif
template <class SC, bool POOL>
__device__ __forceinline__ void kpn_geo_rows_pair_body(const kpn_scene_dev& sc, const kpn_points& ps, const float* __restrict__ wp,
                                                       const int* __restrict__ list, const int* __restrict__ count_ptr,
                                                       int* __restrict__ tickets, float* __restrict__ xscr, const kpn_batch& batch) {
    constexpr int NP = SC::NP;
    if (!kpn_batch_gate(batch, sc, wp)) return;
#if defined(KPN_H2_PAD) && !defined(KPN_SIMT_EMU)
#pragma unroll
    for (int i = 0; i < KPN_H2_PAD; ++i) asm volatile("s_nop 0");
#endif
    const int lane = threadIdx.x & 63;
    const int p = lane & 31, h = lane >> 5;
    const int count = *count_ptr;
    const int ntiles = (count + KPN_TILE - 1) / KPN_TILE;
    int t0, t1;
    if (!kpn_batch_range(batch, ntiles, t0, t1)) return;
    const int nbt = t1 - t0;
    const int nwork = ((nbt + 1) >> 1) * (POOL ? 1 : sc.V);
    const kpn_tile_layout lay(POOL ? 1 : 0, sc.V);
    const uint32_t keep_bits = sc.keep & ((sc.V >= 32) ? 0xFFFFFFFFu : ((1u << sc.V) - 1u));
    const float neg_inv_two_sigma2 = -1.0f / sc.two_sigma2;
    __shared__ __attribute__((aligned(16))) float bias_s[4][128];
    __shared__ __attribute__((aligned(16))) float4 pool_s[POOL ? 4 * 35 * 64 : 1];
    float4* const pst = pool_s + (POOL ? ((threadIdx.x >> 6) * 35 * 64 + lane) : 0);
    {
        const int segs[4] = {SEG_G1_0A, SEG_G1_1, SEG_G1_2, SEG_G1_3};
        for (int i = threadIdx.x; i < 4 * 128; i += blockDim.x) {
            const int sg = i >> 7, k = i & 127;
            const float bscale = (KPN_H2_LOG2ACT && sg < 3) ? KPN_H2_ACT_SCALE : (sg == 3 ? SC::out_up : 1.0f);
            bias_s[sg][k] = k < kpn_seg_bfloats(segs[sg]) ? wp[kpn_seg_boff(segs[sg]) + k] * bscale : 0.0f;
        }
    }
    __syncthreads();
#ifdef KPN_H2_TIMING
    unsigned long long stamp_ = clock64();
#endif
    int nx_ticket = 0;
    int nx_wi = 0;
    int64_t nx_n[2] = {0, 0};
    kpn_point_raw nx_raw[2];
    auto draw_ticket = [&]() { if (lane == 0) nx_ticket = atomicAdd(tickets + 0, 1); };
    auto fetch_list = [&]() {
        nx_wi = __shfl(nx_ticket, 0);
        const int npair = POOL ? nx_wi : nx_wi / sc.V;
#pragma unroll
        for (int t = 0; t < 2; ++t) {
            int64_t ci = (int64_t)(t0 + 2 * npair + t) * KPN_TILE + p;
            if (ci >= count) ci = count - 1;
            nx_n[t] = (int64_t)list[ci];
        }
    };
    auto fetch_points = [&]() {
#pragma unroll
        for (int t = 0; t < 2; ++t) kpn_point_fetch(ps, nx_n[t], nx_raw[t]);
    };
    draw_ticket(); fetch_list(); fetch_points();
#ifndef KPN_SIMT_EMU
    const bool stamp_clk = batch.clk != nullptr && blockIdx.x == 0 && threadIdx.x == 0;
    if (stamp_clk) batch.clk[0] = clock64();
#endif
    for (;;) {
        KPN_H2_STAMP(6);
        const int wi = nx_wi;
        if (wi >= nwork) {
#ifndef KPN_SIMT_EMU
            if (stamp_clk) batch.clk[1] = clock64();
#endif
            return;
        }
        const int pair = POOL ? wi : wi / sc.V;
        const int v_begin = POOL ? 0 : wi - pair * sc.V, v_end = POOL ? sc.V : v_begin + 1;
        const bool has1 = 2 * pair + 1 < nbt;
        float P[2][3], D[2][3];
#pragma unroll
        for (int t = 0; t < 2; ++t) kpn_point_finish(ps, nx_raw[t], P[t], D[t]);
        bool prefetched = false;
        bool first_view = true;
        if constexpr (POOL) {
            pst[32 * 64] = make_float4(P[0][0], P[0][1], P[0][2], 0.0f);
            pst[33 * 64] = make_float4(P[1][0], P[1][1], P[1][2], 0.0f);
        }
      for (int v = v_begin; v < v_end; ++v) {
        const float* tb = sc.table + (size_t)v * KPN_TBL_STRIDE;
        if constexpr (POOL) {
            const float4 p0 = pst[32 * 64], p1 = pst[33 * 64];
            P[0][0] = p0.x; P[0][1] = p0.y; P[0][2] = p0.z; P[1][0] = p1.x; P[1][1] = p1.y; P[1][2] = p1.z;
        }
        kpn_proj q[2];
        float4* dst[2];
#pragma unroll
        for (int t = 0; t < 2; ++t) {
            const int tr = 2 * pair + t;
            q[t] = kpn_project(tb, P[t][0], P[t][1], P[t][2], sc);
            if constexpr (!POOL) dst[t] = reinterpret_cast<float4*>(xscr) + lay.row(tr, v) * 64 + lane;
        }
        if (!((sc.keep >> v) & 1u)) {
            if constexpr (!POOL) {
#pragma unroll
                for (int t = 0; t < 2; ++t) {
                    if (t == 1 && !has1) break;
#pragma unroll
                    for (int k = 0; k < 8; ++k) dst[t][k * 64] = make_float4(0.f, 0.f, 0.f, 0.f);
                }
            }
            continue;
        }
        if constexpr (POOL) pst[34 * 64] = make_float4(kpn_pix_weight_fast(q[0]), kpn_pix_weight_fast(q[1]), 0.0f, 0.0f);
        const bool pf = SC::PREFETCH && !prefetched && (!POOL || (keep_bits >> (v + 1)) == 0u);
        if (pf) draw_ticket();
        KPN_H2_STAMP(0);
        static_assert(kpn_xseg_off(HSEG_G1_0B, NP) == kpn_xseg_off(HSEG_G1_0A, NP) + 12 * kpn_xseg_step_floats(HSEG_G1_0A, NP), "adjacent segments");
        kpn_f32x16 a0[2][4], a1[2][4];
        kpn_u32x4 xa[2][NP], xb[2][NP];
        {
            const float* E = tb + KPN_TBL_EXT;
            float cx[2], cy[2], cz[2];
            kpn_taps tp[2];
#pragma unroll
            for (int t = 0; t < 2; ++t) {
                cx[t] = RADD(kpn_dot3(P[t][0], P[t][1], P[t][2], E[0], E[1], E[2]), E[3]);
                cy[t] = RADD(kpn_dot3(P[t][0], P[t][1], P[t][2], E[4], E[5], E[6]), E[7]);
                cz[t] = RADD(kpn_dot3(P[t][0], P[t][1], P[t][2], E[8], E[9], E[10]), E[11]);
                kpn_load_bias<4>(bias_s[0], h, a0[t]);
                tp[t] = kpn_make_taps(q[t].xn, q[t].yn, sc.g0h, sc.g0w);
            }
            const float* kc = tb + KPN_TBL_KCAM + (12 * h) * 3;
            const float* g0 = sc.geo0 + (size_t)v * sc.g0h * sc.g0w * 64 + 8 * h;
            float fdz[2][2], fw[2][2], fs1[2][2], fc1[2][2];
            float kcv[2][3] = {{kc[0], kc[1], kc[2]}, {kc[3], kc[4], kc[5]}};
            float tdx[2], tdy[2], ty[2], targ[2], ts2[2], tc2[2];
            float4 raw[2][8];
            auto pe_stage = [&](auto ni, auto ti, auto gi) {
                constexpr int n = decltype(ni)::value, t = decltype(ti)::value, g = decltype(gi)::value, b = n & 1;
                if constexpr (g == 0) {
                    tdx[t] = RSUB(cx[t], kcv[b][0]); tdy[t] = RSUB(cy[t], kcv[b][1]); fdz[b][t] = RSUB(cz[t], kcv[b][2]);
                    ty[t] = fdz[b][t] * 0.5f;
                    if constexpr (t == 1 && n + 2 < 12) { kcv[b][0] = kc[(n + 2) * 3 + 0]; kcv[b][1] = kc[(n + 2) * 3 + 1]; kcv[b][2] = kc[(n + 2) * 3 + 2]; }
                } else if constexpr (g == 1) {
                    const float d2 = RADD(RADD(RMUL(tdx[t], tdx[t]), RMUL(tdy[t], tdy[t])), RMUL(fdz[b][t], fdz[b][t]));
                    targ[t] = d2 * neg_inv_two_sigma2;
                } else if constexpr (g == 2) {
                    fw[b][t] = kpn_fast_exp(targ[t]);
#ifndef KPN_SIMT_EMU
                    fs1[b][t] = __builtin_amdgcn_sinf(ty[t]);
#else
                    fs1[b][t] = (float)sin(6.28318530717958647692 * (double)ty[t]);
#endif
                } else if constexpr (g == 3) {
#ifndef KPN_SIMT_EMU
                    fc1[b][t] = __builtin_amdgcn_cosf(ty[t]);
#else
                    fc1[b][t] = (float)cos(6.28318530717958647692 * (double)ty[t]);
#endif
                }
            };
            auto geo_loads = [&](auto si, auto ti, auto fi) {
                constexpr int s = decltype(si)::value, t = decltype(ti)::value, f = decltype(fi)::value;
                const float* gp = g0 + 16 * (s - 12) + 4 * f;
                const kpn_taps& w = tp[t];
                raw[t][4 * f + 0] = *reinterpret_cast<const float4*>(gp + (size_t)w.o00 * 64);
                raw[t][4 * f + 1] = *reinterpret_cast<const float4*>(gp + (size_t)w.o01 * 64);
                raw[t][4 * f + 2] = *reinterpret_cast<const float4*>(gp + (size_t)w.o10 * 64);
                raw[t][4 * f + 3] = *reinterpret_cast<const float4*>(gp + (size_t)w.o11 * 64);
            };
            kpn_static_for<0, 10>([&](auto gi) {
                pe_stage(kpn_ic<0>{}, kpn_ic<0>{}, gi); pe_stage(kpn_ic<0>{}, kpn_ic<1>{}, gi);
            });
            kpn_mfma16_layer2<SC, 16, 4, 0, false, KPN_H2_LOOKAHEAD, kpn_h2_l0_order>(wp + kpn_xseg_off(HSEG_G1_0A, NP), lane,
                [&](auto pi, auto ti, auto ei) -> float {
                    constexpr int s = kpn_h2_l0_order::at(decltype(pi)::value), t = decltype(ti)::value, e = decltype(ei)::value, b = s & 1;
                    if constexpr (s < 12) {
                        if constexpr (e == 0) { return fdz[b][t] * fw[b][t];
                        } else if constexpr (e == 1) { return fs1[b][t] * fw[b][t];
                        } else if constexpr (e == 2) { return fc1[b][t] * fw[b][t];
                        } else if constexpr (e == 3) {
                            ts2[t] = 2.0f * fs1[b][t] * fc1[b][t]; tc2[t] = 1.0f - 2.0f * fs1[b][t] * fs1[b][t];
                            return ts2[t] * fw[b][t];
                        } else if constexpr (e == 4) { return tc2[t] * fw[b][t];
                        } else if constexpr (e == 5) { return (2.0f * ts2[t] * tc2[t]) * fw[b][t];
                        } else if constexpr (e == 6) { return (1.0f - 2.0f * ts2[t] * ts2[t]) * fw[b][t];
                        } else { return 0.0f; }
                    } else {
                        constexpr int f = e / 4, c = e % 4;
                        const kpn_taps& w = tp[t];
                        auto comp = [](const float4& x) { return c == 0 ? x.x : (c == 1 ? x.y : (c == 2 ? x.z : x.w)); };
                        return RADD(RADD(RADD(RMUL(comp(raw[t][4 * f + 0]), w.w00), RMUL(comp(raw[t][4 * f + 1]), w.w01)),
                                         RMUL(comp(raw[t][4 * f + 2]), w.w10)), RMUL(comp(raw[t][4 * f + 3]), w.w11));
                    }
                },
                [&](auto pi, auto ti, auto ji, auto qi) {
                    constexpr int p0 = decltype(pi)::value, t = decltype(ti)::value, j = decltype(ji)::value, qq = decltype(qi)::value;
                    constexpr int g = 3 * j + qq - 2;
                    if constexpr (p0 + 1 < 16 && g >= 0) {
// ... 72 lines not shown
                constexpr int m = decltype(mi)::value;
                if constexpr (m < 2) kpn_load_bias<2>(bias_s[3], h, acc[m]);
            },
            [&](auto ti, auto ei) -> float { return a2[decltype(ti)::value][0][decltype(ei)::value]; },
            a2, xa, xb);
        KPN_H2_STAMP(3);
        kpn_mfma16_layer2<SC, 8, 2, 8, KPN_H2_LOOKAHEAD, false>(wp + kpn_xseg_off(HSEG_G1_3, NP), lane,
            [&](auto si, auto ti, auto ei) -> float {
                constexpr int s = decltype(si)::value, t = decltype(ti)::value, e = decltype(ei)::value;
                return a2[t][s / 2][(s % 2) * 8 + e];
            },
            [](auto, auto, auto, auto) {}, [](auto) {}, [](auto, auto) -> float { return 0.0f; }, acc, xb, xa);
        KPN_H2_STAMP(4);
        prefetched |= pf;
        if constexpr (!POOL) {
#pragma unroll
            for (int t = 0; t < 2; ++t) {
                if (t == 1 && !has1) break;
#pragma unroll
                for (int b = 0; b < 2; ++b)
#pragma unroll
                    for (int qd = 0; qd < 4; ++qd)
                        dst[t][(b * 4 + qd) * 64] =
                            make_float4(acc[t][b][4 * qd + 0] * SC::out_down, acc[t][b][4 * qd + 1] * SC::out_down,
                                        acc[t][b][4 * qd + 2] * SC::out_down, acc[t][b][4 * qd + 3] * SC::out_down);
            }
        } else {
            const bool last_view = (keep_bits >> (v + 1)) == 0u;
            auto welford = [&](auto first_c, auto last_c) {
                constexpr bool FIRST = decltype(first_c)::value, LAST = decltype(last_c)::value;
                const float4 wv4 = pst[34 * 64];
                int lane_late = lane;
#ifndef KPN_SIMT_EMU
                asm volatile("" : "+v"(lane_late));
#endif
#pragma unroll
                for (int t = 0; t < 2; ++t) dst[t] = reinterpret_cast<float4*>(xscr) + lay.tile(2 * pair + t) * 64 + lane_late;
#pragma unroll
                for (int t = 0; t < 2; ++t) {
                    const float4 pw4 = pst[(32 + t) * 64];
                    const float w = t == 0 ? wv4.x : wv4.y;
                    const float wn = pw4.w + w;
                    const float r = wn > 0.0f ? w / wn : 0.0f;
                    const float c = w * (1.0f - r);
                    const float inv = 1.0f / (wn + 1e-6f);
                    const float ms = wn * inv * SC::out_down, vs = inv * (SC::out_down * SC::out_down);
                    const float om2 = wn * (1e-6f * inv) * (1e-6f * inv);
                    const bool store = t == 0 || has1;
#pragma unroll
                    for (int b = 0; b < 2; ++b)
#pragma unroll
                        for (int qd = 0; qd < 4; ++qd) {
                            const int slab = 8 * t + 4 * b + qd;
                            float mu[4], m2[4];
                            if constexpr (FIRST) {
#pragma unroll
                                for (int e = 0; e < 4; ++e) { mu[e] = acc[t][b][4 * qd + e]; m2[e] = 0.0f; }
                            } else {
                                const float4 a = pst[slab * 64], cc = pst[(16 + slab) * 64];
                                const float am[4] = {a.x, a.y, a.z, a.w}, cm[4] = {cc.x, cc.y, cc.z, cc.w};
#pragma unroll
                                for (int e = 0; e < 4; ++e) {
                                    const float d = acc[t][b][4 * qd + e] - am[e];
                                    mu[e] = fmaf(r, d, am[e]);
                                    m2[e] = fmaf(c * d, d, cm[e]);
                                }
                            }
                            if constexpr (!LAST) {
                                pst[slab * 64] = make_float4(mu[0], mu[1], mu[2], mu[3]);
                                if constexpr (!FIRST) pst[(16 + slab) * 64] = make_float4(m2[0], m2[1], m2[2], m2[3]);
                                else pst[(16 + slab) * 64] = make_float4(0.0f, 0.0f, 0.0f, 0.0f);
                            } else if (store) {
                                dst[t][(4 * b + qd) * 64] = make_float4(mu[0] * ms, mu[1] * ms, mu[2] * ms, mu[3] * ms);
                                dst[t][(8 + 4 * b + qd) * 64] = make_float4(fmaf(om2 * mu[0], mu[0], m2[0]) * vs, fmaf(om2 * mu[1], mu[1], m2[1]) * vs,
                                                                            fmaf(om2 * mu[2], mu[2], m2[2]) * vs, fmaf(om2 * mu[3], mu[3], m2[3]) * vs);
                            }
                        }
                    if constexpr (!LAST) pst[(32 + t) * 64] = make_float4(pw4.x, pw4.y, pw4.z, wn);
                }
            };
            if (first_view) { if (last_view) welford(kpn_ic<1>{}, kpn_ic<1>{}); else welford(kpn_ic<1>{}, kpn_ic<0>{}); }
            else { if (last_view) welford(kpn_ic<0>{}, kpn_ic<1>{}); else welford(kpn_ic<0>{}, kpn_ic<0>{}); }
            first_view = false;
        }
      }
        if (!prefetched) { draw_ticket(); fetch_list(); fetch_points(); }
        else if constexpr (POOL) fetch_points();
    }
}

__global__ KPN_H2_BOUNDS void k_geo_rows_h2(kpn_scene_dev sc, kpn_points ps, const float* __restrict__ wp,
                                            const int* __restrict__ list, const int* __restrict__ count_ptr,
                                            int* __restrict__ tickets, float* __restrict__ xscr, kpn_batch batch) {
    kpn_geo_rows_pair_body<kpn_sc_bf16x3, false>(sc, ps, wp, list, count_ptr, tickets, xscr, batch);
}
__global__ KPN_H2_BOUNDS void k_geo_rows_f2(kpn_scene_dev sc, kpn_points ps, const float* __restrict__ wp,
                                            const int* __restrict__ list, const int* __restrict__ count_ptr,
                                            int* __restrict__ tickets, float* __restrict__ xscr, kpn_batch batch) {
    kpn_geo_rows_pair_body<kpn_sc_f16x2, false>(sc, ps, wp, list, count_ptr, tickets, xscr, batch);
}
__global__ KPN_H2_BOUNDS void k_geo_rows_h2p(kpn_scene_dev sc, kpn_points ps, const float* __restrict__ wp,
                                             const int* __restrict__ list, const int* __restrict__ count_ptr,
                                             int* __restrict__ tickets, float* __restrict__ xscr, kpn_batch batch) {
    kpn_geo_rows_pair_body<kpn_sc_bf16x3, true>(sc, ps, wp, list, count_ptr, tickets, xscr, batch);
}
__global__ KPN_H2_BOUNDS void k_geo_rows_f2p(kpn_scene_dev sc, kpn_points ps, const float* __restrict__ wp,
                                             const int* __restrict__ list, const int* __restrict__ count_ptr,
                                             int* __restrict__ tickets, float* __restrict__ xscr, kpn_batch batch) {
    kpn_geo_rows_pair_body<kpn_sc_f16x2, true>(sc, ps, wp, list, count_ptr, tickets, xscr, batch);
}

__global__ __launch_bounds__(256) void k_row_records(kpn_scene_dev sc, kpn_points ps, const float* __restrict__ wp, const int* __restrict__ list,
                                                     const int* __restrict__ count_ptr, float* __restrict__ xscr, kpn_batch batch) {
    const int lane = threadIdx.x & 63, p = lane & 31, tsel = lane >> 5;
    if (batch.cond != KPN_RUN_ALWAYS && !kpn_batch_gate(batch, sc, wp)) return;
    const int count = *count_ptr;
    int t0, t1;
    if (!kpn_batch_range(batch, (count + KPN_TILE - 1) / KPN_TILE, t0, t1)) return;
    const int nbt = t1 - t0;
    const int npairs = (nbt + 1) >> 1;
    const kpn_tile_layout lay(batch.pool, sc.V);
    const int wave = (blockIdx.x * blockDim.x + threadIdx.x) >> 6, nwaves = (gridDim.x * blockDim.x) >> 6;
    auto fetch = [&](int pair, kpn_point_raw& raw) {
        int64_t ci = (int64_t)(t0 + 2 * pair + tsel) * KPN_TILE + p;
        if (ci >= count) ci = count - 1;
        kpn_point_fetch(ps, (int64_t)list[ci], raw);
    };
    kpn_point_raw raw, raw_next;
    if (wave < npairs) fetch(wave, raw);
    for (int pair = wave; pair < npairs; pair += nwaves) {
        if (pair + nwaves < npairs) fetch(pair + nwaves, raw_next);
        const int tr = 2 * pair + tsel;
        float P[3], D[3];
        kpn_point_finish<true>(ps, raw, P, D);
        for (int v = 0; v < sc.V; ++v) {
            const float* tb = sc.table + (size_t)v * KPN_TBL_STRIDE;
            const kpn_proj q = kpn_project<true>(tb, P[0], P[1], P[2], sc);
            float4 a0, a1, b0, b1;
            kpn_row_record_a<true>(sc, tb, v, q, P, D, a0, a1);
            kpn_row_record_b<true>(sc, v, q, b0, b1);
            if (tr < nbt) {
                float4* rec = reinterpret_cast<float4*>(xscr) + lay.rec(tr, v) * 64;
                rec[p] = a0; rec[32 + p] = b0; rec[64 + p] = a1; rec[64 + 32 + p] = b1;
            }
        }
        raw = raw_next;
    }
}

__global__ __launch_bounds__(256) void k_row_records_live(kpn_scene_dev sc, kpn_points ps, const float* __restrict__ wp,
                                                          const int* __restrict__ list, const int* __restrict__ count_ptr,
                                                          const int* __restrict__ tickets, const int* __restrict__ live,
                                                          float* __restrict__ xscr, kpn_batch batch) {
    if (batch.cond != KPN_RUN_ALWAYS && !kpn_batch_gate(batch, sc, wp)) return;
    const int count = *count_ptr;
    int t0, t1;
    if (!kpn_batch_range(batch, (count + KPN_TILE - 1) / KPN_TILE, t0, t1)) return;
    const int nlive = tickets[2];
    const kpn_tile_layout lay(batch.pool, sc.V);
    const int stride = gridDim.x * blockDim.x;
    auto fetch = [&](int e, int& slot, kpn_point_raw& raw) {
        slot = live[e < nlive ? e : nlive - 1];
        kpn_point_fetch(ps, (int64_t)list[t0 * KPN_TILE + slot], raw);
    };
    int e = blockIdx.x * blockDim.x + threadIdx.x;
    const int e_wave = e - (threadIdx.x & 63);
    kpn_point_raw raw, raw_next;
    int slot = 0, slot_next = 0;
// ... 22 lines not shown
```

### keypointnerf_amd/csrc/geo_rows_pair_tu.hip

```cpp
#include "kpn_field_shared.h"
#include "geo_rows_pair_kernels.hip"

#include "geo_rows_pair_launch.h"

#ifdef KPN_PRECISION_PROBE
extern "C" __attribute__((visibility("hidden"))) int kpn_internal_probe_set_mask_pair(unsigned long long m) {
    return hipMemcpyToSymbol(HIP_SYMBOL(kpn_probe_mask_dev), &m, sizeof(m)) != hipSuccess;
}
#endif
#ifdef KPN_H2_TIMING
extern "C" int kpn_h2_timing(unsigned long long* out8) {
    if (hipMemcpyFromSymbol(out8, HIP_SYMBOL(kpn_h2_cycles), 64) != hipSuccess) return 1;
    unsigned long long z[8] = {0, 0, 0, 0, 0, 0, 0, 0};
    return hipMemcpyToSymbol(HIP_SYMBOL(kpn_h2_cycles), z, 64) != hipSuccess;
}
#endif
```

### keypointnerf_amd/csrc/ray_kernels.hip

```cpp
#include "kpn_device.h"

__device__ __forceinline__ int kpn_abs_bits(float a) { return __float_as_int(a) & 0x7fffffff; }
__device__ __forceinline__ int kpn_abs_bits4(int u, const float4& x) {
    const int a = max(kpn_abs_bits(x.x), kpn_abs_bits(x.y)), b = max(kpn_abs_bits(x.z), kpn_abs_bits(x.w));
    return max(u, max(a, b));
}
__device__ __forceinline__ void kpn_note_absmax(float* __restrict__ flags, int u) {
    __shared__ int wmax_s[4];
#pragma unroll
    for (int o = 32; o > 0; o >>= 1) u = max(u, __shfl_xor(u, o));
    if ((threadIdx.x & 63) == 0) wmax_s[threadIdx.x >> 6] = u;
    __syncthreads();
    if (threadIdx.x == 0) {
        u = max(max(wmax_s[0], wmax_s[1]), max(wmax_s[2], wmax_s[3]));
        int* f = reinterpret_cast<int*>(flags);
        if (u > *reinterpret_cast<volatile int*>(f)) atomicMax(f, u);
    }
}

__global__ __launch_bounds__(128) void k_scene_table(int V, int n_kpt, const float* __restrict__ KRT, const float* __restrict__ extrin,
                                                     const float* __restrict__ kpt3d, float* __restrict__ table,
                                                     float* __restrict__ flags) {
    const int v = blockIdx.x, t = threadIdx.x;
    if (v == 0 && t < KPN_SCENE_FLAG_FLOATS) flags[t] = 0.0f;
// ... 65 lines not shown
    const int p0 = (blockIdx.x - v * tiles) * TP;
    const int np = hw - p0 < TP ? hw - p0 : TP;
    const float* src = in + (size_t)v * C * hw + p0;
    int amax = 0;
    if (vec) {
        for (int e = threadIdx.x; e < C * (TP / 4); e += 256) {
            const int c = e / (TP / 4), p = (e % (TP / 4)) * 4;
            if (p < np) {
                const float4 x = *reinterpret_cast<const float4*>(src + (size_t)c * hw + p);
                float* d = tile_s + c * PITCH + p;
                d[0] = x.x; d[1] = x.y; d[2] = x.z; d[3] = x.w;
                amax = kpn_abs_bits4(amax, x);
            }
        }
    } else {
        for (int e = threadIdx.x; e < C * TP; e += 256) {
            const int c = e / TP, p = e % TP;
            if (p < np) {
                const float x = src[(size_t)c * hw + p];
                tile_s[c * PITCH + p] = x;
                amax = max(amax, kpn_abs_bits(x));
            }
        }
    }
    __syncthreads();
    float4* dst = reinterpret_cast<float4*>(out + ((size_t)v * hw + p0) * C);
    for (int o4 = threadIdx.x; o4 < np * (C / 4); o4 += 256) {
        const int p = o4 / (C / 4), c = (o4 % (C / 4)) * 4;
        const float* t = tile_s + c * PITCH + p;
        dst[o4] = make_float4(t[0], t[PITCH], t[2 * PITCH], t[3 * PITCH]);
    }
    kpn_note_absmax(flags, amax);
}

__device__ __forceinline__ void kpn_ray_aabb(const float* __restrict__ bounds, float ox, float oy, float oz, float dx,
                                             float dy, float dz, float& near_o, float& far_o, int& hit) {
    float bmin[3], bmax[3], o[3] = {ox, oy, oz}, d[3] = {dx, dy, dz};
#pragma unroll
    for (int i = 0; i < 3; ++i) {
        bmin[i] = KADD(bounds[i], -0.01f);
        bmax[i] = KADD(bounds[3 + i], 0.01f);
        if (fabsf(d[i]) < 1e-5f) d[i] = 1e-5f;
    }
    int cnt = 0;
    float pint[2][3];
    const float eps = 1e-6f;
#pragma unroll
    for (int s = 0; s < 6; ++s) {
        const int ax = s % 3;
        const float bound = (s < 3) ? bmin[ax] : bmax[ax];
        const float t = KSUB(bound, o[ax]) / d[ax];
        const float p0 = KADD(KMUL(t, d[0]), o[0]), p1 = KADD(KMUL(t, d[1]), o[1]), p2 = KADD(KMUL(t, d[2]), o[2]);
        const int inside = (p0 >= KSUB(bmin[0], eps)) && (p0 <= KADD(bmax[0], eps)) && (p1 >= KSUB(bmin[1], eps)) &&
                           (p1 <= KADD(bmax[1], eps)) && (p2 >= KSUB(bmin[2], eps)) && (p2 <= KADD(bmax[2], eps));
        if (inside) {
            if (cnt < 2) { pint[cnt][0] = p0; pint[cnt][1] = p1; pint[cnt][2] = p2; }
            ++cnt;
        }
    }
    if (cnt == 2) {
        const float nr = sqrtf(kpn_dot3(d[0], d[1], d[2], d[0], d[1], d[2]));
        float dd[2];
#pragma unroll
        for (int k = 0; k < 2; ++k) {
            const float e0 = KSUB(pint[k][0], o[0]), e1 = KSUB(pint[k][1], o[1]), e2 = KSUB(pint[k][2], o[2]);
            dd[k] = sqrtf(kpn_dot3(e0, e1, e2, e0, e1, e2)) / nr;
        }
        near_o = fminf(dd[0], dd[1]); far_o = fmaxf(dd[0], dd[1]); hit = 1;
    } else {
        near_o = 1.0f; far_o = 1.0f; hit = 0;
    }
}

__global__ void k_ray_bbox(int64_t R, const float* __restrict__ bounds, const float* __restrict__ orig,
                           const float* __restrict__ dirs, float* __restrict__ near_o, float* __restrict__ far_o,
                           uint8_t* __restrict__ hit_o) {
    const int64_t r = (int64_t)blockIdx.x * blockDim.x + threadIdx.x;
    if (r >= R) return;
    float n, f; int h;
    kpn_ray_aabb(bounds, orig[0], orig[1], orig[2], dirs[r * 3 + 0], dirs[r * 3 + 1], dirs[r * 3 + 2], n, f, h);
    near_o[r] = n; far_o[r] = f; hit_o[r] = (uint8_t)h;
}

__global__ void k_make_rays(const float* __restrict__ K, const float* __restrict__ RT, float znear, float zfar,
                            const float* __restrict__ bounds, int x0, int y0, int step, int stepy, int nx, int ny,
                            const int* __restrict__ pix, float* __restrict__ dirs, float* __restrict__ cam_pos,
                            float* __restrict__ near_o, float* __restrict__ far_o) {
    const int64_t r = (int64_t)blockIdx.x * blockDim.x + threadIdx.x;
    const int64_t R = (int64_t)nx * ny;
    const double a = K[0], b = K[1], c = K[2], d = K[4], e = K[5], f = K[6], g = K[8], h = K[9], i = K[10];
    const double det = a * (e * i - f * h) - b * (d * i - f * g) + c * (d * h - e * g);
    float iK[9];
    iK[0] = (float)((e * i - f * h) / det); iK[1] = (float)((c * h - b * i) / det); iK[2] = (float)((b * f - c * e) / det);
    iK[3] = (float)((f * g - d * i) / det); iK[4] = (float)((a * i - c * g) / det); iK[5] = (float)((c * d - a * f) / det);
    iK[6] = (float)((d * h - e * g) / det); iK[7] = (float)((b * g - a * h) / det); iK[8] = (float)((a * e - b * d) / det);
    float cp[3];
#pragma unroll
    for (int k = 0; k < 3; ++k)
        cp[k] = -kpn_dot3(RT[0 * 4 + 3], RT[1 * 4 + 3], RT[2 * 4 + 3], RT[0 * 4 + k], RT[1 * 4 + k], RT[2 * 4 + k]);
    if (r == 0) { cam_pos[0] = cp[0]; cam_pos[1] = cp[1]; cam_pos[2] = cp[2]; }
    if (r >= R) return;
    const int iy = (int)(r / nx), ix = (int)(r - (int64_t)iy * nx);
    const float gx = pix ? (float)pix[r * 2 + 0] : (float)(x0 + ix * step);
    const float gy = pix ? (float)pix[r * 2 + 1] : (float)(y0 + iy * stepy), gz = 1.0f;
    float cr[3], cn[3], cf[3];
#pragma unroll
    for (int k = 0; k < 3; ++k) {
        cr[k] = kpn_dot3(gx, gy, gz, iK[k * 3 + 0], iK[k * 3 + 1], iK[k * 3 + 2]);
        cn[k] = kpn_dot3(KMUL(znear, gx), KMUL(znear, gy), KMUL(znear, gz), iK[k * 3 + 0], iK[k * 3 + 1], iK[k * 3 + 2]);
        cf[k] = kpn_dot3(KMUL(zfar, gx), KMUL(zfar, gy), KMUL(zfar, gz), iK[k * 3 + 0], iK[k * 3 + 1], iK[k * 3 + 2]);
    }
    float nr_ = sqrtf(kpn_dot3(cn[0], cn[1], cn[2], cn[0], cn[1], cn[2]));
    float fr_ = sqrtf(kpn_dot3(cf[0], cf[1], cf[2], cf[0], cf[1], cf[2]));
    float w[3];
#pragma unroll
    for (int k = 0; k < 3; ++k) w[k] = kpn_dot3(cr[0], cr[1], cr[2], RT[0 * 4 + k], RT[1 * 4 + k], RT[2 * 4 + k]);
    const float nrm = fmaxf(sqrtf(kpn_dot3(w[0], w[1], w[2], w[0], w[1], w[2])), 1e-12f);
    const float d0 = w[0] / nrm, d1 = w[1] / nrm, d2 = w[2] / nrm;
    dirs[r * 3 + 0] = d0; dirs[r * 3 + 1] = d1; dirs[r * 3 + 2] = d2;
    float z1, z2; int hit;
    kpn_ray_aabb(bounds, cp[0], cp[1], cp[2], d0, d1, d2, z1, z2, hit);
    if (hit && z1 > nr_) nr_ = z1;
    if (hit && z2 < fr_) fr_ = z2;
    near_o[r] = nr_; far_o[r] = fr_;
}

__device__ __forceinline__ float kpn_linspace01(int i, int steps) {
    if (steps == 1) return 0.0f;
    const float step = 1.0f / (float)(steps - 1);
    const int half = steps / 2;
    return (i < half) ? KMUL(step, (float)i) : KSUB(1.0f, KMUL(step, (float)(steps - 1 - i)));
}

__global__ void k_coarse_z(int64_t R, int S, const float* __restrict__ near_i, const float* __restrict__ far_i,
                           const float* __restrict__ u, float* __restrict__ z) {
    const int64_t i = (int64_t)blockIdx.x * blockDim.x + threadIdx.x;
    if (i >= R * S) return;
    const int64_t r = i / S;
    const int s = (int)(i - r * S);
    float t = kpn_linspace01(s, S);
    if (u) {
        const float lo = (s == 0) ? t : KMUL(0.5f, KADD(t, kpn_linspace01(s - 1, S)));
        const float hi = (s == S - 1) ? t : KMUL(0.5f, KADD(kpn_linspace01(s + 1, S), t));
        t = KADD(lo, KMUL(u[i], KSUB(hi, lo)));
    }
    z[i] = KADD(near_i[r], KMUL(KSUB(far_i[r], near_i[r]), t));
}

#define KPN_MAX_PER_LANE 8
template <int PER>
struct kpn_ray_samples { float sig[PER], sd[PER], cr[PER], cg[PER], cb[PER], z[PER], dist[PER]; };
__global__ __launch_bounds__(256) void k_merge_rgba(int64_t n, int S, int Sc, const float* __restrict__ rgba_c, const float* __restrict__ rgba_n,
                                                    const int16_t* __restrict__ src, float* __restrict__ out) {
    const int64_t i = (int64_t)blockIdx.x * blockDim.x + threadIdx.x;
    if (i >= n * S) return;
    const int64_t r = i / S;
    const int id = src[i];
    const float* q = id < Sc ? rgba_c + (r * Sc + id) * 5 : rgba_n + (r * (S - Sc) + (id - Sc)) * 5;
#pragma unroll
    for (int c = 0; c < 5; ++c) out[i * 5 + c] = q[c];
}

template <int PER>
__global__ __launch_bounds__(256) void k_rgba2out(int64_t R, int S, const float* __restrict__ rgba,
                                                  const float* __restrict__ z, float* __restrict__ color,
                                                  float* __restrict__ depth, float* __restrict__ alpha,
                                                  float* __restrict__ contrib, float* __restrict__ sdf,
                                                  const int16_t* __restrict__ src, const float* __restrict__ rgba_new, int Sc) {
    const int lane = threadIdx.x & 63;
    const int64_t wave = ((int64_t)blockIdx.x * blockDim.x + threadIdx.x) >> 6;
    const int64_t nwaves = ((int64_t)gridDim.x * blockDim.x) >> 6;
    const int per = (S + 63) / 64;
    auto load = [&](int64_t r, kpn_ray_samples<PER>& o) {
        const float* zz = z + r * S;
#pragma unroll
        for (int k = 0; k < PER; ++k) {
            const int i = lane * per + k;
            o.sig[k] = 0.0f; o.sd[k] = 0.0f; o.cr[k] = 0.0f; o.cg[k] = 0.0f; o.cb[k] = 0.0f; o.z[k] = 0.0f; o.dist[k] = 0.0f;
            if (k < per && i < S) {
                const float* q;
                if (!src) q = rgba + (r * S + i) * 5;
                else {
                    const int id = src[r * S + i];
                    q = id < Sc ? rgba + (r * Sc + id) * 5 : rgba_new + (r * (S - Sc) + (id - Sc)) * 5;
                }
                o.sig[k] = q[0]; o.sd[k] = q[1]; o.cr[k] = q[2]; o.cg[k] = q[3]; o.cb[k] = q[4];
                o.z[k] = zz[i];
                o.dist[k] = (i + 1 < S) ? (zz[i + 1] - zz[i]) : 1e10f;
            }
        }
    };
    kpn_ray_samples<PER> cur{}, nxt{};
    if (wave < R) load(wave, cur);
    for (int64_t r = wave; r < R; r += nwaves) {
        if (r + nwaves < R) load(r + nwaves, nxt);
        float c[PER];
        float tl = 1.0f;
#pragma unroll
        for (int k = 0; k < PER; ++k) {
            c[k] = 0.0f;
            const int i = lane * per + k;
            if (k < per && i < S) {
                c[k] = 1.0f - expf(-cur.sig[k] * cur.dist[k]);
                tl *= (1.0f - c[k]);
            }
        }
        float incl = tl;
#pragma unroll
        for (int d = 1; d < 64; d <<= 1) {
            const float o = __shfl_up(incl, d);
            if (lane >= d) incl *= o;
        }
        float T = __shfl_up(incl, 1);
        if (lane == 0) T = 1.0f;
        float s_r = 0.f, s_g = 0.f, s_b = 0.f, s_a = 0.f, s_s = 0.f, s_d = 0.f;
#pragma unroll
        for (int k = 0; k < PER; ++k) {
            const int i = lane * per + k;
            if (k < per && i < S) {
                const float cw = c[k] * T;
                T *= (1.0f - c[k]);
                if (contrib) contrib[r * S + i] = cw;
                s_r += cur.cr[k] * cw; s_g += cur.cg[k] * cw; s_b += cur.cb[k] * cw;
                s_a += cw; s_s += cur.sd[k] * cw; s_d += cur.z[k] * cw;
            }
        }
#pragma unroll
        for (int m = 32; m >= 1; m >>= 1) {
            s_r += __shfl_xor(s_r, m); s_g += __shfl_xor(s_g, m); s_b += __shfl_xor(s_b, m);
            s_a += __shfl_xor(s_a, m); s_s += __shfl_xor(s_s, m); s_d += __shfl_xor(s_d, m);
        }
        if (lane == 0) {
            color[r * 3 + 0] = s_r; color[r * 3 + 1] = s_g; color[r * 3 + 2] = s_b;
            alpha[r] = s_a;
            sdf[r] = s_s / (s_a + 1e-8f);
            depth[r] = s_d / (s_a + 1e-8f);
        }
        cur = nxt;
    }
}

__global__ void k_rgba2out_bwd(int64_t R, int S, const float* __restrict__ rgba, const float* __restrict__ z,
                               const float* __restrict__ d_color, const float* __restrict__ d_depth,
                               const float* __restrict__ d_alpha, const float* __restrict__ d_sdf, float* __restrict__ d_rgba) {
    const int64_t r = (int64_t)blockIdx.x * blockDim.x + threadIdx.x;
    if (r >= R) return;
    const float* q = rgba + r * S * 5;
    const float* zz = z + r * S;
    float* dq = d_rgba + r * S * 5;
    double P = 0.0, A64 = 0.0, S64 = 0.0, D64 = 0.0;
    for (int i = 0; i < S; ++i) {
        const float dist = (i + 1 < S) ? (zz[i + 1] - zz[i]) : 1e10f;
        const float tau = q[i * 5 + 0] * dist;
        const float a = -expm1f(-tau);
        const float T = expf(-(float)P);
        const float c = a * T;
        dq[i * 5 + 0] = T;
        P += (double)tau;
        A64 += (double)c; S64 += (double)(q[i * 5 + 1] * c); D64 += (double)(zz[i] * c);
    }
    const float A = (float)A64, Ssum = (float)S64, Dsum = (float)D64;
    const float dc0 = d_color ? d_color[r * 3 + 0] : 0.f, dc1 = d_color ? d_color[r * 3 + 1] : 0.f, dc2 = d_color ? d_color[r * 3 + 2] : 0.f;
    const float dA = d_alpha ? d_alpha[r] : 0.f, dS = d_sdf ? d_sdf[r] : 0.f, dD = d_depth ? d_depth[r] : 0.f;
    const float inv = 1.0f / (A + 1e-8f);
    const float gA = dA - (dS * Ssum + dD * Dsum) * inv * inv;
    double U = 0.0;
    float Tn = expf(-(float)P);
    for (int i = S - 1; i >= 0; --i) {
        const float dist = (i + 1 < S) ? (zz[i + 1] - zz[i]) : 1e10f;
        const float a = -expm1f(-q[i * 5 + 0] * dist);
        const float Ti = dq[i * 5 + 0];
        const float c = a * Ti;
        const float g = dc0 * q[i * 5 + 2] + dc1 * q[i * 5 + 3] + dc2 * q[i * 5 + 4] + gA + dS * q[i * 5 + 1] * inv + dD * zz[i] * inv;
        dq[i * 5 + 0] = (float)((double)Tn * (double)g - U) * dist;
        dq[i * 5 + 1] = c * dS * inv;
        dq[i * 5 + 2] = c * dc0; dq[i * 5 + 3] = c * dc1; dq[i * 5 + 4] = c * dc2;
        U += (double)g * (double)c;
        Tn = Ti;
    }
}

template <int PER>
__global__ __launch_bounds__(256) void k_rgba2out_bwd_w(int64_t R, int S, const float* __restrict__ rgba, const float* __restrict__ z,
                                                        const float* __restrict__ d_color, const float* __restrict__ d_depth,
                                                        const float* __restrict__ d_alpha, const float* __restrict__ d_sdf,
                                                        float* __restrict__ d_rgba) {
    const int lane = threadIdx.x & 63;
    const int64_t r = ((int64_t)blockIdx.x * blockDim.x + threadIdx.x) >> 6;
    if (r >= R) return;
    const int per = (S + 63) / 64;
    const float* zz = z + r * S;
    float sd[PER], cr[PER], cg[PER], cb[PER], zv[PER], dist[PER], tau[PER], e[PER], a[PER], Tk[PER];
    float tl = 0.0f;
#pragma unroll
    for (int k = 0; k < PER; ++k) {
        const int i = lane * per + k;
        sd[k] = cr[k] = cg[k] = cb[k] = zv[k] = dist[k] = 0.0f;
        tau[k] = 0.0f; e[k] = 1.0f; a[k] = 0.0f;
        if (k < per && i < S) {
            const float* q = rgba + (r * S + i) * 5;
            sd[k] = q[1]; cr[k] = q[2]; cg[k] = q[3]; cb[k] = q[4];
            zv[k] = zz[i];
            dist[k] = (i + 1 < S) ? (zz[i + 1] - zz[i]) : 1e10f;
            tau[k] = q[0] * dist[k];
            e[k] = expf(-tau[k]);
            a[k] = 1.0f - e[k];
            tl += tau[k];
        }
    }
    float incl = tl;
#pragma unroll
    for (int d = 1; d < 64; d <<= 1) {
        const float o = __shfl_up(incl, d);
        if (lane >= d) incl += o;
    }
    float P = __shfl_up(incl, 1);
    if (lane == 0) P = 0.0f;
    float A = 0.0f, Ssum = 0.0f, Dsum = 0.0f;
#pragma unroll
    for (int k = 0; k < PER; ++k) {
        Tk[k] = expf(-P);
// ... 263 lines not shown
```

### keypointnerf_amd/lib.py

```python
import ctypes
import os

import torch

_HERE = os.path.dirname(os.path.abspath(__file__))
DEFAULT_LIB = os.path.join(_HERE, "_lib", "libkpnerf_hip.so")

c_f = ctypes.c_float
c_i32 = ctypes.c_int32
c_i64 = ctypes.c_int64
c_p = ctypes.c_void_p
c_sz = ctypes.c_size_t


class SceneDesc(ctypes.Structure):
    _fields_ = [(n, c_i32) for n in ("n_views", "src_h", "src_w", "geo0_h", "geo0_w", "geo1_h", "geo1_w", "tex_h",
                                     "tex_w", "disable_fg_mask")] + \
               [(n, c_f) for n in ("znear", "zfar", "nml_scale", "sigma")] + \
               [(n, c_p) for n in ("KRT", "extrin", "kpt3d", "img", "fg_mask", "geo0", "geo1", "tex")]


class RenderStages(ctypes.Structure):
    _fields_ = [(n, c_p) for n in ("z_coarse", "rgba_coarse", "z_fine", "rgba_fine", "dirs", "cam_pos")]

# ... 78 lines not shown


class ResEncoderDesc(ctypes.Structure):
    _fields_ = [(n, c_i32) for n in ("N", "H", "W", "in_ch", "ngf", "n_down", "n_blocks", "n_up", "out_ch")] + [("eps", c_f)]


class HgFilterDesc(ctypes.Structure):
    _fields_ = [(n, c_i32) for n in ("N", "H", "W", "in_ch", "c_stem", "c2", "c3", "c4", "depth", "c_hd", "out_ch_hd", "out_ch")] + [("eps", c_f)]


class HgFilterParams(ctypes.Structure):
    _fields_ = [("tensors", ctypes.POINTER(c_p)), ("packed", c_p)]


class HgFilterGrads(ctypes.Structure):
    _fields_ = [("tensors", ctypes.POINTER(c_p))]


class ResampleDesc(ctypes.Structure):
    _fields_ = [(n, c_i32) for n in ("N", "h", "w", "C")]


_SIGNATURES = {
    "kpn_abi_version": (ctypes.c_int, []),
    "kpn_last_error": (ctypes.c_char_p, []),
    "kpn_is_device_build": (ctypes.c_int, []),
    "kpn_plain_weight_floats": (c_sz, []),
    "kpn_packed_weight_floats": (c_sz, []),
    "kpn_pack_weights": (ctypes.c_int, [c_p, c_p]),
    "kpn_pack_weights_device": (ctypes.c_int, [c_p, c_p, c_p]),
    "kpn_scene_workspace_bytes": (c_sz, [ctypes.POINTER(SceneDesc)]),
    "kpn_scene_prepare": (ctypes.c_int, [ctypes.POINTER(SceneDesc), c_p, c_p]),
    "kpn_scene_layout": (ctypes.c_int, [ctypes.POINTER(SceneDesc), ctypes.POINTER(c_sz)]),
    "kpn_ray_bbox_intersection": (ctypes.c_int, [c_p, c_p, c_p, c_i64, c_p, c_p, c_p, c_p]),
    "kpn_make_rays": (ctypes.c_int, [c_p, c_p, c_f, c_f, c_p, c_i32, c_i32, c_i32, c_i32, c_i32, c_p, c_p, c_p, c_p, c_p]),
    "kpn_importance_sample": (ctypes.c_int, [c_p, c_p, c_p, c_i64, c_i32, c_i32, c_p, c_p]),
    "kpn_rgba2out": (ctypes.c_int, [c_p, c_p, c_i64, c_i32, c_p, c_p, c_p, c_p, c_p, c_p]),
    "kpn_rgba2out_backward": (ctypes.c_int, [c_p, c_p, c_i64, c_i32, c_p, c_p, c_p, c_p, c_p, c_p]),
    "kpn_geo_rows_backward_workspace_bytes": (c_sz, [c_i64, c_i32]),
    "kpn_geo_rows_backward": (ctypes.c_int, [ctypes.POINTER(SceneDesc), c_p, c_p, c_i64, c_p, ctypes.c_uint32, c_p, c_p, c_p,
                                             c_p, c_p, c_sz, c_p]),
    "kpn_query_backward_geometry_workspace_bytes": (c_sz, [c_i64, c_i32]),
    "kpn_query_backward_geometry": (ctypes.c_int, [ctypes.POINTER(SceneDesc), c_p, c_p, c_i64, c_p, c_i32, ctypes.c_uint32, c_p,
                                                   ctypes.c_float, c_p, c_p, c_p, c_p, c_p, c_sz, c_p]),
    "kpn_query_backward_workspace_bytes": (c_sz, [c_i64, c_i32]),
    "kpn_query_backward": (ctypes.c_int, [ctypes.POINTER(SceneDesc), c_p, c_p, c_i64, c_p, c_p, c_i32, ctypes.c_uint32, c_p,
                                          ctypes.c_float, c_p, c_p, c_p, c_p, c_p, c_p, c_sz, c_p]),
    "kpn_render_rays_train_backward_workspace_bytes": (c_sz, [ctypes.POINTER(SceneDesc), ctypes.POINTER(RenderArgs)]),
    "kpn_render_rays_train_backward": (ctypes.c_int, [ctypes.POINTER(SceneDesc), c_p, c_p, ctypes.POINTER(RenderArgs),
                                                      ctypes.POINTER(TrainArgs), ctypes.POINTER(RenderGrads), c_p, c_p, c_p, c_p,
                                                      c_p, c_sz, c_p]),
    "kpn_geo_rows_backward_workspace_bytes_kpt": (c_sz, [c_i64, c_i32]),
    "kpn_geo_rows_backward_kpt": (ctypes.c_int, [ctypes.POINTER(SceneDesc), c_p, c_p, c_i64, c_p, ctypes.c_uint32, c_p, c_p, c_p,
                                                 c_p, c_p, c_i32, c_p, c_sz, c_p]),
    "kpn_query_backward_workspace_bytes_kpt": (c_sz, [c_i64, c_i32]),
    "kpn_query_backward_kpt": (ctypes.c_int, [ctypes.POINTER(SceneDesc), c_p, c_p, c_i64, c_p, c_p, c_i32, ctypes.c_uint32, c_p,
                                              ctypes.c_float, c_p, c_p, c_p, c_p, c_p, c_p, c_i32, c_p, c_sz, c_p]),
    "kpn_render_rays_train_backward_workspace_bytes_kpt": (c_sz, [ctypes.POINTER(SceneDesc), ctypes.POINTER(RenderArgs)]),
    "kpn_render_rays_train_backward_kpt": (ctypes.c_int, [ctypes.POINTER(SceneDesc), c_p, c_p, ctypes.POINTER(RenderArgs),
                                                          ctypes.POINTER(TrainArgs), ctypes.POINTER(RenderGrads), c_p, c_p, c_p, c_p,
                                                          c_p, c_i32, c_p, c_sz, c_p]),
    "kpn_render_rays_train_backward_kept_kpt": (ctypes.c_int, [ctypes.POINTER(SceneDesc), c_p, c_p, ctypes.POINTER(RenderArgs),
                                                               ctypes.POINTER(TrainArgs), ctypes.POINTER(RenderGrads), c_p, c_p, c_p,
                                                               c_p, c_p, c_i32, c_p, c_sz, c_p, c_sz, c_p]),
    "kpn_set_geo_rows_mode": (ctypes.c_int, [c_i32]),
    "kpn_get_geo_rows_mode": (ctypes.c_int, []),
    "kpn_packed_f16_range_check": (ctypes.c_int, [c_p, c_p, c_p]),
    "kpn_set_fuse_mode": (ctypes.c_int, [c_i32]),
    "kpn_get_fuse_mode": (ctypes.c_int, []),
    "kpn_set_density_first": (ctypes.c_int, [c_i32]),
    "kpn_get_density_first": (ctypes.c_int, []),
    "kpn_density_stats": (ctypes.c_int, [c_p, c_p, c_p, c_i32]),
    "kpn_density_first_passes": (ctypes.c_int, [c_p, c_p, c_i32]),
    "kpn_bwd_profile_enable": (ctypes.c_int, [c_i32]),
    "kpn_bwd_profile_collect": (ctypes.c_int, [c_p, c_p, c_p, c_p, c_p]),
    "kpn_set_range_guard": (ctypes.c_int, [c_i32]),
    "kpn_get_range_guard": (ctypes.c_int, []),
    "kpn_range_guard_count": (ctypes.c_int, [c_p, c_p]),
    "kpn_ssim_scratch_bytes": (c_sz, [c_i32, c_i32]),
    "kpn_ssim": (ctypes.c_int, [c_p, c_p, c_i32, c_i32, c_i32, c_i32, c_i32, c_i32, c_p, c_p, c_p]),
    "kpn_query_workspace_bytes": (c_sz, [c_i64, c_i32]),
    "kpn_query": (ctypes.c_int, [ctypes.POINTER(SceneDesc), c_p, c_p, c_i64, c_p, c_p, c_i32, c_p, c_p, c_p, c_sz, c_p]),
    "kpn_render_workspace_bytes": (c_sz, [ctypes.POINTER(SceneDesc), ctypes.POINTER(RenderArgs)]),
    "kpn_render_rays": (ctypes.c_int, [ctypes.POINTER(SceneDesc), c_p, c_p, ctypes.POINTER(RenderArgs), c_p, c_sz, c_p]),
    "kpn_render_rays_train": (ctypes.c_int, [ctypes.POINTER(SceneDesc), c_p, c_p, ctypes.POINTER(RenderArgs),
                                             ctypes.POINTER(TrainArgs), c_p, c_sz, c_p]),
    "kpn_frame_to_rgb8": (ctypes.c_int, [c_p, c_i32, c_i32, c_i32, c_p, c_p]),
    "kpn_mse_psnr": (ctypes.c_int, [c_p, c_p, c_i64, c_p, c_p, c_p]),
    "kpn_flops_per_point": (ctypes.c_double, [c_i32]),
    "kpn_flops_per_row": (ctypes.c_double, []),
    "kpn_profile_enable": (ctypes.c_int, [c_i32]),
    "kpn_render_rays_train_state_bytes": (c_sz, [ctypes.POINTER(SceneDesc), ctypes.POINTER(RenderArgs)]),
    "kpn_render_rays_train_keep": (ctypes.c_int, [ctypes.POINTER(SceneDesc), c_p, c_p, ctypes.POINTER(RenderArgs),
                                                  ctypes.POINTER(TrainArgs), c_p, c_sz, c_p]),
    "kpn_render_rays_train_backward_kept": (ctypes.c_int, [ctypes.POINTER(SceneDesc), c_p, c_p, ctypes.POINTER(RenderArgs),
                                                           ctypes.POINTER(TrainArgs), ctypes.POINTER(RenderGrads), c_p, c_p, c_p, c_p,
                                                           c_p, c_sz, c_p, c_sz, c_p]),
    "kpn_pix_l1_loss": (ctypes.c_int, [c_p, c_p, ctypes.c_int64, ctypes.c_float, c_p, c_p, c_p, c_p]),
    "kpn_train_loss_workspace_bytes": (c_sz, [c_i64]),
    "kpn_train_loss": (ctypes.c_int, [ctypes.POINTER(TrainLossArgs), c_p, c_p]),
    "kpn_profile_collect": (ctypes.c_int, [c_p, c_p, c_p]),
    "kpn_profile_collect2": (ctypes.c_int, [c_p, c_p, c_p, c_p]),
    "kpn_profile_collect3": (ctypes.c_int, [c_p, c_p, c_p, c_p, c_p]),
    "kpn_row_scratch_cap_bytes": (ctypes.c_size_t, []),
    "kpn_set_row_scratch_cap_bytes": (ctypes.c_int, [ctypes.c_size_t]),
    "kpn_selftest_mfma": (ctypes.c_int, [c_p, c_p, c_p]),
    "kpn_vgg_plain_floats": (c_sz, []),
    "kpn_vgg_packed_floats": (c_sz, []),
    "kpn_vgg_pack_device": (ctypes.c_int, [c_p, c_p, c_p]),
    "kpn_vgg_workspace_bytes": (c_sz, [c_i32, c_i32, c_i32]),
    "kpn_vgg_stage_floats": (c_sz, [c_i32, c_i32, c_i32]),
    "kpn_vgg_loss": (ctypes.c_int, [c_p, c_p, c_i32, c_i32, c_i32, c_p, c_p, c_p, c_p, c_f, c_p, c_p, c_p, c_p, c_sz, c_p]),
    "kpn_geo_encoder_plain_floats": (c_sz, [c_i32, c_i32]),
    "kpn_geo_encoder_packed_floats": (c_sz, [c_i32, c_i32]),
    "kpn_geo_encoder_pack_device": (ctypes.c_int, [c_p, c_p, c_i32, c_i32, c_p]),
    "kpn_geo_encoder_workspace_bytes": (c_sz, [c_i32] * 6),
    "kpn_geo_encoder_stage_floats": (c_sz, [c_i32] * 6),
    "kpn_geo_encoder_stage_info": (ctypes.c_int, [c_i32] * 7 + [ctypes.c_char_p, c_i32, ctypes.POINTER(c_i64), ctypes.POINTER(c_i32)]),
    "kpn_geo_encode": (ctypes.c_int, [c_p] + [c_i32] * 6 + [c_p, c_f, c_p, c_p, c_p, c_p, c_sz, c_p]),
    "kpn_tex_encoder_plain_floats": (c_sz, [c_i32] * 5),
    "kpn_tex_encoder_packed_floats": (c_sz, [c_i32] * 5),
    "kpn_tex_encoder_pack_device": (ctypes.c_int, [c_p, c_p] + [c_i32] * 5 + [c_p]),
    "kpn_tex_encoder_workspace_bytes": (c_sz, [c_i32] * 9),
    "kpn_tex_encoder_stage_floats": (c_sz, [c_i32] * 9),
    "kpn_tex_encoder_stage_info": (ctypes.c_int, [c_i32] * 10 + [ctypes.c_char_p, c_i32, ctypes.POINTER(c_i64), ctypes.POINTER(c_i32)]),
    "kpn_tex_encode": (ctypes.c_int, [c_p] + [c_i32] * 9 + [c_p, c_f, c_p, c_p, c_p, c_sz, c_p]),
    "kpn_fold_norm_floats": (c_sz, []),
    "kpn_fold_params": (ctypes.c_int, [ctypes.POINTER(ParamTable), c_p, c_p, c_p]),
    "kpn_fold_params_backward": (ctypes.c_int, [ctypes.POINTER(ParamTable), c_p, c_p, ctypes.POINTER(ParamTable), c_i32, c_p]),
    "kpn_adam_step": (ctypes.c_int, [ctypes.POINTER(AdamArgs), c_p]),
    "kpn_plain_weight_floats_shape": (c_sz, [ctypes.POINTER(FieldShape)]),
    "kpn_widen_plain": (ctypes.c_int, [ctypes.POINTER(FieldShape), c_p, c_p, c_p]),
    "kpn_narrow_plain_grad": (ctypes.c_int, [ctypes.POINTER(FieldShape), c_p, c_p, c_i32, c_p]),
    "kpn_scene_prepare_kpt": (ctypes.c_int, [ctypes.POINTER(SceneDesc), c_i32, c_p, c_p]),
    "kpn_fold_params_shape": (ctypes.c_int, [ctypes.POINTER(FieldShape), ctypes.POINTER(ParamTable), c_p, c_p, c_p]),
    "kpn_fold_params_backward_shape": (ctypes.c_int, [ctypes.POINTER(FieldShape), ctypes.POINTER(ParamTable), c_p, c_p,
                                                      ctypes.POINTER(ParamTable), c_i32, c_p]),
    "kpn_conv2d_packed_floats": (c_sz, [ctypes.POINTER(Conv2dDesc)]),
    "kpn_conv2d_pack_device": (ctypes.c_int, [ctypes.POINTER(Conv2dDesc), c_p, c_p, c_p]),
    "kpn_conv2d_workspace_bytes": (c_sz, [ctypes.POINTER(Conv2dDesc)]),
    "kpn_conv2d_wgrad_ranges": (c_i32, [ctypes.POINTER(Conv2dDesc)]),
    "kpn_conv2d_forward": (ctypes.c_int, [ctypes.POINTER(Conv2dDesc), c_p, c_p, c_p, c_p, c_p, c_sz, c_p]),
    "kpn_conv2d_backward": (ctypes.c_int, [ctypes.POINTER(Conv2dDesc), c_p, c_p, c_p, c_p, c_p, c_p, c_p, c_sz, c_p]),
    "kpn_conv2d_ex_packed_floats": (c_sz, [ctypes.POINTER(Conv2dDesc), c_i32]),
    "kpn_conv2d_ex_pack_device": (ctypes.c_int, [ctypes.POINTER(Conv2dDesc), c_i32, c_p, c_p, c_p]),
    "kpn_conv2d_ex_workspace_bytes": (c_sz, [ctypes.POINTER(Conv2dDesc), c_i32]),
    "kpn_conv2d_ex_wgrad_ranges": (c_i32, [ctypes.POINTER(Conv2dDesc), c_i32]),
    "kpn_conv2d_ex_forward": (ctypes.c_int, [ctypes.POINTER(Conv2dDesc), c_i32, c_p, c_p, c_p, c_p, c_p, c_sz, c_p]),
    "kpn_conv2d_ex_backward": (ctypes.c_int, [ctypes.POINTER(Conv2dDesc), c_i32, c_p, c_p, c_p, c_p, c_p, c_p, c_p, c_sz, c_p]),
    "kpn_conv2d_s2_packed_floats": (c_sz, [ctypes.POINTER(Conv2dS2Desc)]),
    "kpn_conv2d_s2_pack_device": (ctypes.c_int, [ctypes.POINTER(Conv2dS2Desc), c_p, c_p, c_p]),
    "kpn_conv2d_s2_workspace_bytes": (c_sz, [ctypes.POINTER(Conv2dS2Desc)]),
    "kpn_conv2d_s2_wgrad_ranges": (c_i32, [ctypes.POINTER(Conv2dS2Desc)]),
    "kpn_conv2d_s2_forward": (ctypes.c_int, [ctypes.POINTER(Conv2dS2Desc), c_p, c_p, c_p, c_p, c_p, c_sz, c_p]),
    "kpn_conv2d_s2_backward": (ctypes.c_int, [ctypes.POINTER(Conv2dS2Desc), c_p, c_p, c_p, c_p, c_p, c_p, c_p, c_sz, c_p]),
    "kpn_conv2d_rp_packed_floats": (c_sz, [ctypes.POINTER(Conv2dRpDesc)]),
    "kpn_conv2d_rp_pack_device": (ctypes.c_int, [ctypes.POINTER(Conv2dRpDesc), c_p, c_p, c_p]),
    "kpn_conv2d_rp_workspace_bytes": (c_sz, [ctypes.POINTER(Conv2dRpDesc)]),
    "kpn_conv2d_rp_wgrad_ranges": (c_i32, [ctypes.POINTER(Conv2dRpDesc)]),
    "kpn_conv2d_rp_forward": (ctypes.c_int, [ctypes.POINTER(Conv2dRpDesc), c_p, c_p, c_p, c_p, c_p, c_sz, c_p]),
    "kpn_conv2d_rp_backward": (ctypes.c_int, [ctypes.POINTER(Conv2dRpDesc), c_p, c_p, c_p, c_p, c_p, c_p, c_p, c_sz, c_p]),
    "kpn_group_norm_stats_floats": (c_sz, [ctypes.POINTER(GroupNormDesc)]),
    "kpn_group_norm_workspace_bytes": (c_sz, [ctypes.POINTER(GroupNormDesc)]),
    "kpn_group_norm_forward": (ctypes.c_int, [ctypes.POINTER(GroupNormDesc), c_p, c_p, c_p, c_p, c_p, c_p, c_sz, c_p]),
    "kpn_group_norm_backward": (ctypes.c_int, [ctypes.POINTER(GroupNormDesc), c_p, c_p, c_p, c_p, c_p, c_p, c_p, c_p, c_sz, c_p]),
    "kpn_conv_block_workspace_bytes": (c_sz, [ctypes.POINTER(ConvBlockDesc)]),
# ... 75 lines not shown
```

Baseline: 13.23 million.

## Track sample validity as bitmasks and skip masked samples in compositing

```diff
diff --git a/include/kpnerf.h b/include/kpnerf.h
--- a/include/kpnerf.h
+++ b/include/kpnerf.h
@@ -137,6 +137,7 @@
 enum { KPN_FUSE_DEFAULT = 0, KPN_FUSE_F32 = 1, KPN_FUSE_F16X2 = 2 };
 
 size_t kpn_render_workspace_bytes(const kpn_scene_desc* desc, const kpn_render_args* args);
+int kpn_render_keeps_valid_words(const kpn_scene_desc* desc, const kpn_render_args* args);
 int kpn_render_rays(const kpn_scene_desc* desc, const void* scene_ws, const float* packed_weights,
                     const kpn_render_args* args, void* workspace, size_t workspace_bytes, void* stream);
 
diff --git a/keypointnerf_amd/csrc/api_backward.hip b/keypointnerf_amd/csrc/api_backward.hip
--- a/keypointnerf_amd/csrc/api_backward.hip
+++ b/keypointnerf_amd/csrc/api_backward.hip
@@ -203,7 +203,7 @@
         } else {
             const int ppt = mask_points_per_thread(n);
             KPN_LAUNCH(k_mask_compact, grid1d(n, 256 * ppt), dim3(256), stream, sc, ps, n, 0, 1, ppt, wp + kpn_scalar_off(), (float*)nullptr,
-                       (uint8_t*)nullptr, list, count);
+                       (uint8_t*)nullptr, list, count, (unsigned long long*)nullptr);
         }
         KPN_LAUNCH(k_bwd_rows, dim3(1), dim3(1), stream, vcount, V, rows_dev);
         bwd_prof_pass(vcount, V, p.keep_mask, stream);
diff --git a/keypointnerf_amd/csrc/api_field.hip b/keypointnerf_amd/csrc/api_field.hip
--- a/keypointnerf_amd/csrc/api_field.hip
+++ b/keypointnerf_amd/csrc/api_field.hip
@@ -149,6 +149,7 @@
     kpn_points points; int64_t N = 0; int mode = 0;
     float* out = nullptr; uint8_t* valid = nullptr; void* ws = nullptr;
     bool lean = false, keep_rows = false, allow_pool = false; int rows_sel = 0, fuse_sel = 0;
+    unsigned long long* valid_words = nullptr;
 };
 struct FieldLaunch { const kpn_scene_dev& sc; const kpn_points& ps; const float* wp; int *list, *count, *live; float* xscr; void* stream; };
 kpn_batch make_batch(int index, int tiles_cap, bool pool, int cond = KPN_RUN_ALWAYS, int* bad = nullptr, int* redone = nullptr) {
@@ -192,7 +193,9 @@
                         reinterpret_cast<float*>(base + L.xscr), stream};
     hipMemsetAsync(count, 0, kCounterBytes, (hipStream_t)stream);
     const int ppt = mask_points_per_thread(p.N);
-    KPN_LAUNCH(k_mask_compact, grid1d(p.N, 256 * ppt), dim3(256), stream, sc, ps, p.N, p.mode, (int)p.lean, ppt, wp + kpn_scalar_off(), p.out, p.valid, f.list, count);
+    KPN_REQUIRE(!p.valid_words || (p.lean && p.mode == 1 && p.out), "validity words: lean eval_func passes only");
+    KPN_LAUNCH(k_mask_compact, grid1d(p.N, 256 * ppt), dim3(256), stream, sc, ps, p.N, p.mode, (int)p.lean, ppt, wp + kpn_scalar_off(), p.out, p.valid, f.list, count,
+               p.valid_words);
     if (p.keep_rows && L.nbatch > 1) return fail(KPN_EWORKSPACE, "a pass whose rows a backward call reads again must fit the row scratch");
     const bool guard = range_guard() && p.out && (rmode == 3 || fmode == 1);
     int* redone = guard ? redone_counter() : nullptr;
diff --git a/keypointnerf_amd/csrc/api_render.hip b/keypointnerf_amd/csrc/api_render.hip
--- a/keypointnerf_amd/csrc/api_render.hip
+++ b/keypointnerf_amd/csrc/api_render.hip
@@ -56,6 +56,24 @@
     L.total = c.o;
     return L;
 }
+struct ValidWords { size_t c = 0, f = 0; bool ok = false; };
+ValidWords place_valid_words(const RenderLayout& L, int64_t Sc, int64_t Sfine, bool fine, bool reuse) {
+    ValidWords v;
+    Carver c;
+    c.o = L.color;
+    v.c = c.take((size_t)((L.chunk * Sc + 63) / 64) * 8);
+    if (fine && reuse) v.f = c.take((size_t)((L.chunk * Sfine + 63) / 64) * 8);
+    else v.f = L.src;
+    v.ok = c.o <= L.sdf + align_up((size_t)L.chunk * 4, 256);
+    return v;
+}
+ValidWords eval_valid_words(const RenderLayout& L, const kpn_render_args* a) {
+    const bool reuse = a->fine && !env_flag("KPN_NO_COARSE_REUSE");
+    const int64_t Sf = a->fine ? a->n_fine : 0;
+    ValidWords v = place_valid_words(L, a->n_coarse, reuse ? Sf : a->n_coarse + Sf, a->fine != 0, reuse);
+    v.ok = v.ok && !env_flag("KPN_NO_VALID_WORDS");
+    return v;
+}
 int check_render(const kpn_render_args* a) {
     KPN_REQUIRE(a != nullptr, "render args null");
     KPN_REQUIRE(a->K && a->RT && a->bounds, "null camera/bounds");
@@ -107,6 +125,11 @@
     return render_layout(d, a).total;
 }
 
+extern "C" int kpn_render_keeps_valid_words(const kpn_scene_desc* d, const kpn_render_args* a) {
+    if (check_desc(d) != KPN_OK || check_render(a) != KPN_OK) return -1;
+    return eval_valid_words(render_layout(d, a), a).ok ? 1 : 0;
+}
+
 static void launch_fine_samples(void* stream, int64_t n, int Sc, int Sf, const float* zc, const float* contrib,
                                 const float* u, float* zf, float* znew, int16_t* src) {
     const bool small = Sc <= 64 && Sf <= 64;
@@ -118,9 +141,10 @@
         KPN_LAUNCH(k_fine_samples_w<false>, grid, dim3(256), stream, n, Sc, Sf, zc, contrib, u, zf, znew, src);
 }
 
-static void launch_make_rays(void* stream, const kpn_render_args* a, const int* pix, int step_y, const RayView& rays) {
+static void launch_make_rays(void* stream, const kpn_render_args* a, const int* pix, int step_y, const RayView& rays, float* zc = nullptr,
+                             int64_t zc_rays = 0) {
     KPN_LAUNCH(k_make_rays, grid1d((int64_t)a->nx * a->ny, 256), dim3(256), stream, a->K, a->RT, a->znear, a->zfar, a->bounds, (int)a->x0, (int)a->y0,
-               (int)a->step, step_y, (int)a->nx, (int)a->ny, pix, rays.dirs, rays.cam_pos, rays.nearv, rays.farv);
+               (int)a->step, step_y, (int)a->nx, (int)a->ny, pix, rays.dirs, rays.cam_pos, rays.nearv, rays.farv, zc, (int)a->n_coarse, zc_rays);
 }
 
 static int render_impl(const kpn_scene_desc* d, const void* scene_ws, const float* wp, const kpn_render_args* a,
@@ -139,25 +163,41 @@
     const int64_t R = (int64_t)a->nx * a->ny;
     const int Sc = a->n_coarse, Sf = a->fine ? a->n_fine : 0, Sfull = Sc + Sf;
     const float std_ = t ? t->rand_noise_std : 0.0f;
-    launch_make_rays(stream, a, t ? (const int*)t->pix : (const int*)nullptr, (int)(a->step_y > 0 ? a->step_y : a->step), rays);
+    const bool reuse_now = (t == nullptr) && a->fine && !env_flag("KPN_NO_COARSE_REUSE");
+    const ValidWords vwo = eval_valid_words(L, a);
+    const bool words = (t == nullptr) && vwo.ok;
+    launch_make_rays(stream, a, t ? (const int*)t->pix : (const int*)nullptr, (int)(a->step_y > 0 ? a->step_y : a->step), rays,
+                     words ? k.zc : nullptr, R < L.chunk ? R : L.chunk);
     for (int64_t r0 = 0; r0 < R; r0 += L.chunk) {
         const int64_t n = (R - r0) < L.chunk ? (R - r0) : L.chunk;
         const float* dirs = rays.dirs + r0 * 3;
         const PlanarChunk pl{stream, r0, n, R};
-        KPN_LAUNCH(k_coarse_z, grid1d(n * Sc, 256), dim3(256), stream, n, Sc, (const float*)(rays.nearv + r0),
-                   (const float*)(rays.farv + r0), t ? t->u_coarse + r0 * Sc : (const float*)nullptr, k.zc);
-        const bool reuse = (t == nullptr) && a->fine && !env_flag("KPN_NO_COARSE_REUSE");
-        auto field = [&](const float* z, int S, const float* noise, float* out) {
+        if (!words || r0 > 0)
+            KPN_LAUNCH(k_coarse_z, grid1d(n * Sc, 256), dim3(256), stream, n, Sc, (const float*)(rays.nearv + r0),
+                       (const float*)(rays.farv + r0), t ? t->u_coarse + r0 * Sc : (const float*)nullptr, k.zc);
+        const bool reuse = reuse_now;
+        auto field = [&](const float* z, int S, const float* noise, float* out, unsigned long long* vw) {
             FieldPass p;
             p.points = kpn_points{nullptr, nullptr, rays.cam_pos, dirs, z, S, noise, std_};
             p.N = n * S; p.mode = 1; p.out = out; p.ws = k.query_c; p.lean = true; p.allow_pool = t == nullptr;
-            p.rows_sel = a->rows_kernel; p.fuse_sel = a->fuse_kernel;
+            p.rows_sel = a->rows_kernel; p.fuse_sel = a->fuse_kernel; p.valid_words = vw;
             return run_field(sc, wp, p, stream);
         };
         sc.keep = t ? t->keep_coarse : 0xFFFFFFFFu;
-        if (int e = field(k.zc, Sc, std_ != 0.0f ? t->noise_coarse + r0 * Sc : nullptr, k.rgba_c)) return e;
-        if (int e = kpn_rgba2out(k.rgba_c, k.zc, n, Sc, color, depth, alpha, k.contrib, sdf, stream)) return e;
+        unsigned long long *vw_c = words ? at<unsigned long long>(ws, vwo.c) : nullptr, *vw_f = words ? at<unsigned long long>(ws, vwo.f) : nullptr;
+        CompositeExtras x;
+        if (words) { x.vw = vw_c; x.vw_new = vw_f; x.nml_scale = sc.nml_scale; x.plane_r0 = r0; x.plane_R = R; }
+        if (int e = field(k.zc, Sc, std_ != 0.0f ? t->noise_coarse + r0 * Sc : nullptr, k.rgba_c, vw_c)) return e;
+        if (!words) { if (int e = kpn_rgba2out(k.rgba_c, k.zc, n, Sc, color, depth, alpha, k.contrib, sdf, stream)) return e; }
+        else {
+            launch_rgba2out(stream, n, Sc, k.rgba_c, k.zc, a->tex_fg, a->depth, a->alpha, k.contrib, nullptr, nullptr, nullptr, 0, x);
+            if (int e = check_launch("kpn_render_rays")) return e;
+        }
         const kpn_render_stages* st = a->stages;
+        auto fill_masked = [&](int64_t N, const unsigned long long* vw, float* rgba) {
+            KPN_LAUNCH(k_fill_masked, grid1d(N, 256), dim3(256), stream, N, vw, sc.nml_scale, rgba);
+        };
+        if (words && st && (st->rgba_coarse || (st->rgba_fine && reuse))) fill_masked(n * Sc, vw_c, k.rgba_c);
         auto copy_out = [&](float* dst, const float* src_, size_t floats) {
             (void)hipMemcpyAsync(dst, src_, floats * sizeof(float), hipMemcpyDeviceToDevice, (hipStream_t)stream);
         };
@@ -165,19 +205,29 @@
         if (st && st->cam_pos && r0 == 0) copy_out(st->cam_pos, rays.cam_pos, 3);
         if (st && st->z_coarse) copy_out(st->z_coarse + r0 * Sc, k.zc, (size_t)n * Sc);
         if (st && st->rgba_coarse) copy_out(st->rgba_coarse + r0 * Sc * 5, k.rgba_c, (size_t)n * Sc * 5);
-        pl.store(a->tex_fg, color, 3);
-        pl.store(a->depth, depth, 1);
-        pl.store(a->alpha, alpha, 1);
+        if (!words) {
+            pl.store(a->tex_fg, color, 3);
+            pl.store(a->depth, depth, 1);
+            pl.store(a->alpha, alpha, 1);
+        }
         if (!a->fine) continue;
         launch_fine_samples(stream, n, Sc, Sf, k.zc, k.contrib, t ? t->u_fine + r0 * Sf : (const float*)nullptr, k.zf, reuse ? zn : nullptr,
                             reuse ? src : nullptr);
         sc.keep = t ? t->keep_fine : 0xFFFFFFFFu;
         if (reuse) {
-            if (int e = field(zn, Sf, nullptr, rgba_n)) return e;
-            if (int e = rgba2out_merged(k.rgba_c, rgba_n, src, k.zf, n, Sc, Sf, color, depth, alpha, sdf, stream)) return e;
+            if (int e = field(zn, Sf, nullptr, rgba_n, vw_f)) return e;
+            if (!words) { if (int e = rgba2out_merged(k.rgba_c, rgba_n, src, k.zf, n, Sc, Sf, color, depth, alpha, sdf, stream)) return e; }
+            else if (int e = rgba2out_merged(k.rgba_c, rgba_n, src, k.zf, n, Sc, Sf, a->tex_fg_fine, a->depth_fine, a->alpha_fine, a->sdf, stream, x)) return e;
+            if (words && st && st->rgba_fine) fill_masked(n * Sf, vw_f, rgba_n);
         } else {
-            if (int e = field(k.zf, Sfull, std_ != 0.0f ? t->noise_fine + r0 * Sfull : nullptr, k.rgba_f)) return e;
-            if (int e = kpn_rgba2out(k.rgba_f, k.zf, n, Sfull, color, depth, alpha, nullptr, sdf, stream)) return e;
+            if (int e = field(k.zf, Sfull, std_ != 0.0f ? t->noise_fine + r0 * Sfull : nullptr, k.rgba_f, vw_f)) return e;
+            if (!words) { if (int e = kpn_rgba2out(k.rgba_f, k.zf, n, Sfull, color, depth, alpha, nullptr, sdf, stream)) return e; }
+            else {
+                x.vw = vw_f;
+                launch_rgba2out(stream, n, Sfull, k.rgba_f, k.zf, a->tex_fg_fine, a->depth_fine, a->alpha_fine, nullptr, a->sdf, nullptr, nullptr, 0, x);
+                if (int e = check_launch("kpn_render_rays")) return e;
+                if (st && st->rgba_fine) fill_masked(n * Sfull, vw_f, k.rgba_f);
+            }
         }
         if (st && st->z_fine) copy_out(st->z_fine + r0 * Sfull, k.zf, (size_t)n * Sfull);
         if (st && st->rgba_fine) {
@@ -185,6 +235,7 @@
                                   (const int16_t*)src, st->rgba_fine + r0 * Sfull * 5);
             else copy_out(st->rgba_fine + r0 * Sfull * 5, k.rgba_f, (size_t)n * Sfull * 5);
         }
+        if (words) continue;
         pl.store(a->tex_fg_fine, color, 3);
         pl.store(a->depth_fine, depth, 1);
         pl.store(a->alpha_fine, alpha, 1);
diff --git a/keypointnerf_amd/csrc/api_scene.hip b/keypointnerf_amd/csrc/api_scene.hip
--- a/keypointnerf_amd/csrc/api_scene.hip
+++ b/keypointnerf_amd/csrc/api_scene.hip
@@ -95,7 +95,7 @@
     KPN_REQUIRE(K && RT && bounds && dirs && cam_pos && near_o && far_o, "null pointer");
     KPN_REQUIRE(nx > 0 && ny > 0 && step > 0, "bad pixel grid");
     KPN_LAUNCH(k_make_rays, grid1d((int64_t)nx * ny, 256), dim3(256), stream, K, RT, znear, zfar, bounds, (int)x0, (int)y0,
-               (int)step, (int)step, (int)nx, (int)ny, (const int*)nullptr, dirs, cam_pos, near_o, far_o);
+               (int)step, (int)step, (int)nx, (int)ny, (const int*)nullptr, dirs, cam_pos, near_o, far_o, (float*)nullptr, 0, (int64_t)0);
     return check_launch("kpn_make_rays");
 }
 
@@ -109,15 +109,23 @@
     return check_launch("kpn_importance_sample");
 }
 
+struct CompositeExtras { const unsigned long long *vw = nullptr, *vw_new = nullptr; float nml_scale = 1.0f; int64_t plane_r0 = 0, plane_R = 0; };
 static void launch_rgba2out(void* stream, int64_t R, int S, const float* rgba, const float* z, float* color, float* depth,
-                            float* alpha, float* contrib, float* sdf, const int16_t* src, const float* rgba_new, int Sc) {
+                            float* alpha, float* contrib, float* sdf, const int16_t* src, const float* rgba_new, int Sc,
+                            const CompositeExtras& x = CompositeExtras()) {
     const int64_t blocks = (R + 3) / 4;
     const dim3 grid((unsigned)(blocks < 8192 ? blocks : 8192));
     const int per = (S + 63) / 64;
-    if (per <= 1) KPN_LAUNCH(k_rgba2out<1>, grid, dim3(256), stream, R, S, rgba, z, color, depth, alpha, contrib, sdf, src, rgba_new, Sc);
-    else if (per <= 2) KPN_LAUNCH(k_rgba2out<2>, grid, dim3(256), stream, R, S, rgba, z, color, depth, alpha, contrib, sdf, src, rgba_new, Sc);
-    else if (per <= 4) KPN_LAUNCH(k_rgba2out<4>, grid, dim3(256), stream, R, S, rgba, z, color, depth, alpha, contrib, sdf, src, rgba_new, Sc);
-    else KPN_LAUNCH(k_rgba2out<KPN_MAX_PER_LANE>, grid, dim3(256), stream, R, S, rgba, z, color, depth, alpha, contrib, sdf, src, rgba_new, Sc);
+#define KPN_RGBA2OUT_ARGS R, S, rgba, z, color, depth, alpha, contrib, sdf, src, rgba_new, Sc, x.vw, x.vw_new, x.nml_scale, x.plane_r0, x.plane_R
+    if (x.vw) {
+        if (per <= 1) KPN_LAUNCH((k_rgba2out<1, true>), grid, dim3(256), stream, KPN_RGBA2OUT_ARGS);
+        else if (per <= 2) KPN_LAUNCH((k_rgba2out<2, true>), grid, dim3(256), stream, KPN_RGBA2OUT_ARGS);
+        else KPN_LAUNCH((k_rgba2out<4, true>), grid, dim3(256), stream, KPN_RGBA2OUT_ARGS);
+    } else if (per <= 1) KPN_LAUNCH((k_rgba2out<1, false>), grid, dim3(256), stream, KPN_RGBA2OUT_ARGS);
+    else if (per <= 2) KPN_LAUNCH((k_rgba2out<2, false>), grid, dim3(256), stream, KPN_RGBA2OUT_ARGS);
+    else if (per <= 4) KPN_LAUNCH((k_rgba2out<4, false>), grid, dim3(256), stream, KPN_RGBA2OUT_ARGS);
+    else KPN_LAUNCH((k_rgba2out<KPN_MAX_PER_LANE, false>), grid, dim3(256), stream, KPN_RGBA2OUT_ARGS);
+#undef KPN_RGBA2OUT_ARGS
 }
 
 extern "C" int kpn_rgba2out(const float* rgba, const float* z, int64_t R, int32_t S, float* color, float* depth,
@@ -129,8 +137,8 @@
     return check_launch("kpn_rgba2out");
 }
 static int rgba2out_merged(const float* rgba_c, const float* rgba_n, const int16_t* src, const float* z, int64_t R, int Sc, int Sf,
-                           float* color, float* depth, float* alpha, float* sdf, void* stream) {
-    launch_rgba2out(stream, R, Sc + Sf, rgba_c, z, color, depth, alpha, nullptr, sdf, src, rgba_n, Sc);
+                           float* color, float* depth, float* alpha, float* sdf, void* stream, const CompositeExtras& x = CompositeExtras()) {
+    launch_rgba2out(stream, R, Sc + Sf, rgba_c, z, color, depth, alpha, nullptr, sdf, src, rgba_n, Sc, x);
     return check_launch("kpn_render_rays");
 }
 
diff --git a/keypointnerf_amd/csrc/field_kernels.hip b/keypointnerf_amd/csrc/field_kernels.hip
--- a/keypointnerf_amd/csrc/field_kernels.hip
+++ b/keypointnerf_amd/csrc/field_kernels.hip
@@ -5,7 +5,7 @@
 __global__ __launch_bounds__(256) void k_mask_compact(kpn_scene_dev sc, kpn_points ps, int64_t N, int mode, int lean, int ppt,
                                                       const float* __restrict__ wscalars, float* __restrict__ out,
                                                       uint8_t* __restrict__ valid, int* __restrict__ list,
-                                                      int* __restrict__ count) {
+                                                      int* __restrict__ count, unsigned long long* __restrict__ vwords) {
     __shared__ unsigned long long mask_s[KPN_MASK_PPT][4];
     __shared__ int off_s[KPN_MASK_PPT][4];
     const int lane = threadIdx.x & 63, w = threadIdx.x >> 6;
@@ -33,7 +33,7 @@
             }
             is_valid = all_in && all_fg && ((sc.keep & ((1u << sc.V) - 1u)) != 0u);
             if (valid) valid[n] = (uint8_t)is_valid;
-            if (!is_valid && out) {
+            if (!is_valid && out && !vwords) {
                 float* o = out + n * 5;
                 if (mode == 1) { o[0] = 0.0f; o[1] = 0.1f / sc.nml_scale; }
                 else { o[0] = wscalars[1]; o[1] = wscalars[2]; }
@@ -41,7 +41,10 @@
             }
         }
         const unsigned long long m = __ballot(is_valid);
-        if (lane == 0) mask_s[k][w] = m;
+        if (lane == 0) {
+            mask_s[k][w] = m;
+            if (vwords && n < N) vwords[n >> 6] = m;
+        }
     }
     __syncthreads();
     if (threadIdx.x == 0) {
diff --git a/keypointnerf_amd/csrc/geo_rows_pair_kernels.hip b/keypointnerf_amd/csrc/geo_rows_pair_kernels.hip
--- a/keypointnerf_amd/csrc/geo_rows_pair_kernels.hip
+++ b/keypointnerf_amd/csrc/geo_rows_pair_kernels.hip
@@ -331,9 +331,12 @@
 };
 #ifdef KPN_H2_TIMING
 __device__ unsigned long long kpn_h2_cycles[8];
+__device__ unsigned long long kpn_h2_counts[2];
 #define KPN_H2_STAMP(i) do { const unsigned long long now_ = clock64(); if (blockIdx.x == 3 && threadIdx.x == 64) atomicAdd(&kpn_h2_cycles[i], now_ - stamp_); stamp_ = now_; } while (0)
+#define KPN_H2_COUNT(i) do { if (blockIdx.x == 3 && threadIdx.x == 64) atomicAdd(&kpn_h2_counts[i], 1ull); } while (0)
 #else
 #define KPN_H2_STAMP(i) ((void)0)
+#define KPN_H2_COUNT(i) ((void)0)
 #endif
 #ifndef KPN_SIMT_EMU
 #ifdef KPN_H2_NUM_VGPR
@@ -456,7 +459,7 @@
         if constexpr (POOL) pst[34 * 64] = make_float4(kpn_pix_weight_fast(q[0]), kpn_pix_weight_fast(q[1]), 0.0f, 0.0f);
         const bool pf = SC::PREFETCH && !prefetched && (!POOL || (keep_bits >> (v + 1)) == 0u);
         if (pf) draw_ticket();
-        KPN_H2_STAMP(0);
+        KPN_H2_STAMP(first_view ? 0 : 7);
         static_assert(kpn_xseg_off(HSEG_G1_0B, NP) == kpn_xseg_off(HSEG_G1_0A, NP) + 12 * kpn_xseg_step_floats(HSEG_G1_0A, NP), "adjacent segments");
         kpn_f32x16 a0[2][4], a1[2][4];
         kpn_u32x4 xa[2][NP], xb[2][NP];
@@ -695,8 +698,11 @@
             if (first_view) { if (last_view) welford(kpn_ic<1>{}, kpn_ic<1>{}); else welford(kpn_ic<1>{}, kpn_ic<0>{}); }
             else { if (last_view) welford(kpn_ic<0>{}, kpn_ic<1>{}); else welford(kpn_ic<0>{}, kpn_ic<0>{}); }
             first_view = false;
-        }
+            KPN_H2_STAMP(5);
+        }
+        KPN_H2_COUNT(0);
       }
+        KPN_H2_COUNT(1);
         if (!prefetched) { draw_ticket(); fetch_list(); fetch_points(); }
         else if constexpr (POOL) fetch_points();
     }
diff --git a/keypointnerf_amd/csrc/geo_rows_pair_tu.hip b/keypointnerf_amd/csrc/geo_rows_pair_tu.hip
--- a/keypointnerf_amd/csrc/geo_rows_pair_tu.hip
+++ b/keypointnerf_amd/csrc/geo_rows_pair_tu.hip
@@ -14,4 +14,9 @@
     unsigned long long z[8] = {0, 0, 0, 0, 0, 0, 0, 0};
     return hipMemcpyToSymbol(HIP_SYMBOL(kpn_h2_cycles), z, 64) != hipSuccess;
 }
+extern "C" int kpn_h2_timing_counts(unsigned long long* out2) {
+    if (hipMemcpyFromSymbol(out2, HIP_SYMBOL(kpn_h2_counts), 16) != hipSuccess) return 1;
+    unsigned long long z[2] = {0, 0};
+    return hipMemcpyToSymbol(HIP_SYMBOL(kpn_h2_counts), z, 16) != hipSuccess;
+}
 #endif
diff --git a/keypointnerf_amd/csrc/ray_kernels.hip b/keypointnerf_amd/csrc/ray_kernels.hip
--- a/keypointnerf_amd/csrc/ray_kernels.hip
+++ b/keypointnerf_amd/csrc/ray_kernels.hip
@@ -171,12 +171,17 @@
     near_o[r] = n; far_o[r] = f; hit_o[r] = (uint8_t)h;
 }
 
-__global__ void k_make_rays(const float* __restrict__ K, const float* __restrict__ RT, float znear, float zfar,
-                            const float* __restrict__ bounds, int x0, int y0, int step, int stepy, int nx, int ny,
-                            const int* __restrict__ pix, float* __restrict__ dirs, float* __restrict__ cam_pos,
-                            float* __restrict__ near_o, float* __restrict__ far_o) {
-    const int64_t r = (int64_t)blockIdx.x * blockDim.x + threadIdx.x;
-    const int64_t R = (int64_t)nx * ny;
+__device__ __forceinline__ float kpn_linspace01(int i, int steps) {
+    if (steps == 1) return 0.0f;
+    const float step = 1.0f / (float)(steps - 1);
+    const int half = steps / 2;
+    return (i < half) ? KMUL(step, (float)i) : KSUB(1.0f, KMUL(step, (float)(steps - 1 - i)));
+}
+
+__device__ __forceinline__ void kpn_make_ray(const float* __restrict__ K, const float* __restrict__ RT, float znear, float zfar,
+                                             const float* __restrict__ bounds, int x0, int y0, int step, int stepy, int nx,
+                                             const int* __restrict__ pix, int64_t r, float* __restrict__ dirs, float* __restrict__ cam_pos,
+                                             float* __restrict__ near_o, float* __restrict__ far_o, float& nr_, float& fr_) {
     const double a = K[0], b = K[1], c = K[2], d = K[4], e = K[5], f = K[6], g = K[8], h = K[9], i = K[10];
     const double det = a * (e * i - f * h) - b * (d * i - f * g) + c * (d * h - e * g);
     float iK[9];
@@ -188,7 +193,6 @@
     for (int k = 0; k < 3; ++k)
         cp[k] = -kpn_dot3(RT[0 * 4 + 3], RT[1 * 4 + 3], RT[2 * 4 + 3], RT[0 * 4 + k], RT[1 * 4 + k], RT[2 * 4 + k]);
     if (r == 0) { cam_pos[0] = cp[0]; cam_pos[1] = cp[1]; cam_pos[2] = cp[2]; }
-    if (r >= R) return;
     const int iy = (int)(r / nx), ix = (int)(r - (int64_t)iy * nx);
     const float gx = pix ? (float)pix[r * 2 + 0] : (float)(x0 + ix * step);
     const float gy = pix ? (float)pix[r * 2 + 1] : (float)(y0 + iy * stepy), gz = 1.0f;
@@ -199,8 +203,8 @@
         cn[k] = kpn_dot3(KMUL(znear, gx), KMUL(znear, gy), KMUL(znear, gz), iK[k * 3 + 0], iK[k * 3 + 1], iK[k * 3 + 2]);
         cf[k] = kpn_dot3(KMUL(zfar, gx), KMUL(zfar, gy), KMUL(zfar, gz), iK[k * 3 + 0], iK[k * 3 + 1], iK[k * 3 + 2]);
     }
-    float nr_ = sqrtf(kpn_dot3(cn[0], cn[1], cn[2], cn[0], cn[1], cn[2]));
-    float fr_ = sqrtf(kpn_dot3(cf[0], cf[1], cf[2], cf[0], cf[1], cf[2]));
+    nr_ = sqrtf(kpn_dot3(cn[0], cn[1], cn[2], cn[0], cn[1], cn[2]));
+    fr_ = sqrtf(kpn_dot3(cf[0], cf[1], cf[2], cf[0], cf[1], cf[2]));
     float w[3];
 #pragma unroll
     for (int k = 0; k < 3; ++k) w[k] = kpn_dot3(cr[0], cr[1], cr[2], RT[0 * 4 + k], RT[1 * 4 + k], RT[2 * 4 + k]);
@@ -214,11 +218,30 @@
     near_o[r] = nr_; far_o[r] = fr_;
 }
 
-__device__ __forceinline__ float kpn_linspace01(int i, int steps) {
-    if (steps == 1) return 0.0f;
-    const float step = 1.0f / (float)(steps - 1);
-    const int half = steps / 2;
-    return (i < half) ? KMUL(step, (float)i) : KSUB(1.0f, KMUL(step, (float)(steps - 1 - i)));
+__global__ void k_make_rays(const float* __restrict__ K, const float* __restrict__ RT, float znear, float zfar,
+                            const float* __restrict__ bounds, int x0, int y0, int step, int stepy, int nx, int ny,
+                            const int* __restrict__ pix, float* __restrict__ dirs, float* __restrict__ cam_pos,
+                            float* __restrict__ near_o, float* __restrict__ far_o, float* __restrict__ zc, int Sc, int64_t zc_rays) {
+    const int64_t r = (int64_t)blockIdx.x * blockDim.x + threadIdx.x;
+    const int64_t R = (int64_t)nx * ny;
+    if (zc) {
+        float nr_ = 0.0f, fr_ = 0.0f;
+        if (r < R) kpn_make_ray(K, RT, znear, zfar, bounds, x0, y0, step, stepy, nx, pix, r, dirs, cam_pos, near_o, far_o, nr_, fr_);
+        const int lane = threadIdx.x & 63;
+        const int64_t rb = r - lane;
+        const float t0 = kpn_linspace01(lane < Sc ? lane : 0, Sc), t1 = kpn_linspace01(lane + 64 < Sc ? lane + 64 : 0, Sc);
+        for (int j = 0; j < 64; ++j) {
+            const float nj = __shfl(nr_, j), fj = __shfl(fr_, j);
+            if (rb + j >= zc_rays) break;
+            float* row = zc + (rb + j) * Sc;
+            if (lane < Sc) row[lane] = KADD(nj, KMUL(KSUB(fj, nj), t0));
+            if (lane + 64 < Sc) row[lane + 64] = KADD(nj, KMUL(KSUB(fj, nj), t1));
+        }
+        return;
+    }
+    if (r >= R) return;
+    float nr_, fr_;
+    kpn_make_ray(K, RT, znear, zfar, bounds, x0, y0, step, stepy, nx, pix, r, dirs, cam_pos, near_o, far_o, nr_, fr_);
 }
 
 __global__ void k_coarse_z(int64_t R, int S, const float* __restrict__ near_i, const float* __restrict__ far_i,
@@ -238,7 +261,9 @@
 
 #define KPN_MAX_PER_LANE 8
 template <int PER>
-struct kpn_ray_samples { float sig[PER], sd[PER], cr[PER], cg[PER], cb[PER], z[PER], dist[PER]; };
+struct kpn_ray_samples { float sig[PER], sd[PER], cr[PER], cg[PER], cb[PER], z[PER], dist[PER]; int live; };
+template <int PER>
+struct kpn_ray_index { int id[PER]; unsigned long long w[PER]; };
 __global__ __launch_bounds__(256) void k_merge_rgba(int64_t n, int S, int Sc, const float* __restrict__ rgba_c, const float* __restrict__ rgba_n,
                                                     const int16_t* __restrict__ src, float* __restrict__ out) {
     const int64_t i = (int64_t)blockIdx.x * blockDim.x + threadIdx.x;
@@ -250,82 +275,145 @@
     for (int c = 0; c < 5; ++c) out[i * 5 + c] = q[c];
 }
 
-template <int PER>
+__global__ __launch_bounds__(256) void k_fill_masked(int64_t N, const unsigned long long* __restrict__ vw, float nml_scale, float* __restrict__ out) {
+    const int64_t j = (int64_t)blockIdx.x * blockDim.x + threadIdx.x;
+    if (j >= N || ((vw[j >> 6] >> (j & 63)) & 1ull)) return;
+    float* o = out + j * 5;
+    o[0] = 0.0f; o[1] = 0.1f / nml_scale; o[2] = 0.0f; o[3] = 0.0f; o[4] = 0.0f;
+}
+
+template <int PER, bool WORDS>
 __global__ __launch_bounds__(256) void k_rgba2out(int64_t R, int S, const float* __restrict__ rgba,
                                                   const float* __restrict__ z, float* __restrict__ color,
                                                   float* __restrict__ depth, float* __restrict__ alpha,
                                                   float* __restrict__ contrib, float* __restrict__ sdf,
-                                                  const int16_t* __restrict__ src, const float* __restrict__ rgba_new, int Sc) {
+                                                  const int16_t* __restrict__ src, const float* __restrict__ rgba_new, int Sc,
+                                                  const unsigned long long* __restrict__ vw,
+                                                  const unsigned long long* __restrict__ vw_new, float nml_scale,
+                                                  int64_t plane_r0, int64_t plane_R) {
+    const float sd_masked = 0.1f / nml_scale;
     const int lane = threadIdx.x & 63;
     const int64_t wave = ((int64_t)blockIdx.x * blockDim.x + threadIdx.x) >> 6;
     const int64_t nwaves = ((int64_t)gridDim.x * blockDim.x) >> 6;
     const int per = (S + 63) / 64;
-    auto load = [&](int64_t r, kpn_ray_samples<PER>& o) {
+    auto locate = [&](int64_t r, int i, int id, int64_t& j, const float*& base, const unsigned long long*& words) {
+        j = r * S + i; base = rgba; words = vw;
+        if (src) {
+            if (id < Sc) j = r * Sc + id;
+            else { j = r * (S - Sc) + (id - Sc); base = rgba_new; words = vw_new; }
+        }
+    };
+    auto load_ids = [&](int64_t r, kpn_ray_index<PER>& x) {
+#pragma unroll
+        for (int k = 0; k < PER; ++k) {
+            const int i = lane * per + k;
+            x.id[k] = (src && k < per && i < S) ? (int)src[r * S + i] : 0;
+        }
+    };
+    auto load_words = [&](int64_t r, kpn_ray_index<PER>& x) {
+#pragma unroll
+        for (int k = 0; k < PER; ++k) {
+            const int i = lane * per + k;
+            x.w[k] = ~0ull;
+            if (WORDS && k < per && i < S) {
+                int64_t j; const float* base; const unsigned long long* words;
+                locate(r, i, x.id[k], j, base, words);
+                x.w[k] = words[j >> 6];
+            }
+        }
+    };
+    auto load = [&](int64_t r, const kpn_ray_index<PER>& x, kpn_ray_samples<PER>& o) {
         const float* zz = z + r * S;
+        o.live = 0;
 #pragma unroll
         for (int k = 0; k < PER; ++k) {
             const int i = lane * per + k;
             o.sig[k] = 0.0f; o.sd[k] = 0.0f; o.cr[k] = 0.0f; o.cg[k] = 0.0f; o.cb[k] = 0.0f; o.z[k] = 0.0f; o.dist[k] = 0.0f;
             if (k < per && i < S) {
-                const float* q;
-                if (!src) q = rgba + (r * S + i) * 5;
-                else {
-                    const int id = src[r * S + i];
-                    q = id < Sc ? rgba + (r * Sc + id) * 5 : rgba_new + (r * (S - Sc) + (id - Sc)) * 5;
-                }
-                o.sig[k] = q[0]; o.sd[k] = q[1]; o.cr[k] = q[2]; o.cg[k] = q[3]; o.cb[k] = q[4];
-                o.z[k] = zz[i];
-                o.dist[k] = (i + 1 < S) ? (zz[i + 1] - zz[i]) : 1e10f;
+                int64_t j; const float* base; const unsigned long long* words;
+                locate(r, i, x.id[k], j, base, words);
+                if (!WORDS || ((x.w[k] >> (j & 63)) & 1ull)) {
+                    const float* q = base + j * 5;
+                    o.sig[k] = q[0]; o.sd[k] = q[1]; o.cr[k] = q[2]; o.cg[k] = q[3]; o.cb[k] = q[4];
+                    o.z[k] = zz[i];
+                    o.dist[k] = (i + 1 < S) ? (zz[i + 1] - zz[i]) : 1e10f;
+                    o.live = 1;
+                } else o.sd[k] = sd_masked;
             }
         }
     };
     kpn_ray_samples<PER> cur{}, nxt{};
-    if (wave < R) load(wave, cur);
+    kpn_ray_index<PER> xa{}, xb{}, xc{};
+    if (wave < R) load_ids(wave, xc);
+    if constexpr (WORDS) {
+        if (wave + nwaves < R) load_ids(wave + nwaves, xa);
+        if (wave + 2 * nwaves < R) load_ids(wave + 2 * nwaves, xb);
+    }
+    if (wave < R) { load_words(wave, xc); load(wave, xc, cur); }
+    if constexpr (WORDS) { if (wave + nwaves < R) load_words(wave + nwaves, xa); }
     for (int64_t r = wave; r < R; r += nwaves) {
-        if (r + nwaves < R) load(r + nwaves, nxt);
-        float c[PER];
-        float tl = 1.0f;
-#pragma unroll
-        for (int k = 0; k < PER; ++k) {
-            c[k] = 0.0f;
-            const int i = lane * per + k;
-            if (k < per && i < S) {
-                c[k] = 1.0f - expf(-cur.sig[k] * cur.dist[k]);
-                tl *= (1.0f - c[k]);
-            }
-        }
-        float incl = tl;
-#pragma unroll
-        for (int d = 1; d < 64; d <<= 1) {
-            const float o = __shfl_up(incl, d);
-            if (lane >= d) incl *= o;
-        }
-        float T = __shfl_up(incl, 1);
-        if (lane == 0) T = 1.0f;
+        if constexpr (WORDS) {
+            if (r + nwaves < R) load(r + nwaves, xa, nxt);
+            if (r + 2 * nwaves < R) load_words(r + 2 * nwaves, xb);
+            if (r + 3 * nwaves < R) load_ids(r + 3 * nwaves, xc);
+        } else if (r + nwaves < R) { load_ids(r + nwaves, xa); load(r + nwaves, xa, nxt); }
         float s_r = 0.f, s_g = 0.f, s_b = 0.f, s_a = 0.f, s_s = 0.f, s_d = 0.f;
-#pragma unroll
-        for (int k = 0; k < PER; ++k) {
-            const int i = lane * per + k;
-            if (k < per && i < S) {
-                const float cw = c[k] * T;
-                T *= (1.0f - c[k]);
-                if (contrib) contrib[r * S + i] = cw;
-                s_r += cur.cr[k] * cw; s_g += cur.cg[k] * cw; s_b += cur.cb[k] * cw;
-                s_a += cw; s_s += cur.sd[k] * cw; s_d += cur.z[k] * cw;
-            }
-        }
-#pragma unroll
-        for (int m = 32; m >= 1; m >>= 1) {
-            s_r += __shfl_xor(s_r, m); s_g += __shfl_xor(s_g, m); s_b += __shfl_xor(s_b, m);
-            s_a += __shfl_xor(s_a, m); s_s += __shfl_xor(s_s, m); s_d += __shfl_xor(s_d, m);
+        if (WORDS && !__any(cur.live)) {
+            if (contrib) {
+#pragma unroll
+                for (int k = 0; k < PER; ++k) {
+                    const int i = lane * per + k;
+                    if (k < per && i < S) contrib[r * S + i] = 0.0f;
+                }
+            }
+        } else {
+            float c[PER];
+            float tl = 1.0f;
+#pragma unroll
+            for (int k = 0; k < PER; ++k) {
+                c[k] = 0.0f;
+                const int i = lane * per + k;
+                if (k < per && i < S) {
+                    c[k] = 1.0f - expf(-cur.sig[k] * cur.dist[k]);
+                    tl *= (1.0f - c[k]);
+                }
+            }
+            float incl = tl;
+#pragma unroll
+            for (int d = 1; d < 64; d <<= 1) {
+                const float o = __shfl_up(incl, d);
+                if (lane >= d) incl *= o;
+            }
+            float T = __shfl_up(incl, 1);
+            if (lane == 0) T = 1.0f;
+#pragma unroll
+            for (int k = 0; k < PER; ++k) {
+                const int i = lane * per + k;
+                if (k < per && i < S) {
+                    const float cw = c[k] * T;
+                    T *= (1.0f - c[k]);
+                    if (contrib) contrib[r * S + i] = cw;
+                    s_r += cur.cr[k] * cw; s_g += cur.cg[k] * cw; s_b += cur.cb[k] * cw;
+                    s_a += cw; s_s += cur.sd[k] * cw; s_d += cur.z[k] * cw;
+                }
+            }
+#pragma unroll
+            for (int m = 32; m >= 1; m >>= 1) {
+                s_r += __shfl_xor(s_r, m); s_g += __shfl_xor(s_g, m); s_b += __shfl_xor(s_b, m);
+                s_a += __shfl_xor(s_a, m); s_s += __shfl_xor(s_s, m); s_d += __shfl_xor(s_d, m);
+            }
         }
         if (lane == 0) {
-            color[r * 3 + 0] = s_r; color[r * 3 + 1] = s_g; color[r * 3 + 2] = s_b;
-            alpha[r] = s_a;
-            sdf[r] = s_s / (s_a + 1e-8f);
-            depth[r] = s_d / (s_a + 1e-8f);
+            const int64_t ro = plane_r0 + r;
+            if (plane_R > 0) {
+                if (color) { color[ro] = s_r; color[plane_R + ro] = s_g; color[2 * plane_R + ro] = s_b; }
+            } else { color[r * 3 + 0] = s_r; color[r * 3 + 1] = s_g; color[r * 3 + 2] = s_b; }
+            if (alpha) alpha[ro] = s_a;
+            if (sdf) sdf[ro] = s_s / (s_a + 1e-8f);
+            if (depth) depth[ro] = s_d / (s_a + 1e-8f);
         }
         cur = nxt;
+        if constexpr (WORDS) { xa = xb; xb = xc; }
     }
 }
 
diff --git a/keypointnerf_amd/lib.py b/keypointnerf_amd/lib.py
--- a/keypointnerf_amd/lib.py
+++ b/keypointnerf_amd/lib.py
@@ -184,6 +184,7 @@
     "kpn_query_workspace_bytes": (c_sz, [c_i64, c_i32]),
     "kpn_query": (ctypes.c_int, [ctypes.POINTER(SceneDesc), c_p, c_p, c_i64, c_p, c_p, c_i32, c_p, c_p, c_p, c_sz, c_p]),
     "kpn_render_workspace_bytes": (c_sz, [ctypes.POINTER(SceneDesc), ctypes.POINTER(RenderArgs)]),
+    "kpn_render_keeps_valid_words": (ctypes.c_int, [ctypes.POINTER(SceneDesc), ctypes.POINTER(RenderArgs)]),
     "kpn_render_rays": (ctypes.c_int, [ctypes.POINTER(SceneDesc), c_p, c_p, ctypes.POINTER(RenderArgs), c_p, c_sz, c_p]),
     "kpn_render_rays_train": (ctypes.c_int, [ctypes.POINTER(SceneDesc), c_p, c_p, ctypes.POINTER(RenderArgs),
                                              ctypes.POINTER(TrainArgs), c_p, c_sz, c_p]),
```

After: 13.44 million, median of 6. 1.02x the previous value.
